# penn-graphics-research/HOT

Measured on AMD Instinct MI355X. Metric: ms per nonlinear (L-BFGS) iteration; P2G+G2P Mparticles/s; achieved HBM GB/s vs roofline, lower is better.
Workload: dtype f64; 1 GPU; C2: one 63^3-cell cube x 8 ppc (63^3 cells per GPU), fixed-corotated E=50000 nu=0.3, dx=0.01, dt=1/24, -lsolver 3 -mg_level 3 -smoother 5 -coarseSolver 2 --project --linesearch --bcproject --usecn -cneps 1e-7; particles_per_gpu=2000376, particles_total=2000376, nodes_total=267563, levels=3, parallelism=1 GPU

## Files before the change

hot_amd/csrc/mg_gs.hip:

```cpp
#include "hot_impl.h"

namespace hot {

#ifdef HOT_AB_KERNELS
#include "ab_src/mg_gs_ab1.hip"
#endif

template <class T, int SB>
struct GsLds {
    static constexpr int TRI = SB * (SB - 1) / 2 + 1;
    static constexpr size_t bytes = (size_t)9 * TRI * sizeof(T) + SB * 3 * sizeof(T) + 5 * SB * sizeof(int32_t);
};
template <class T>
struct GsWinv {
    static constexpr int img_elems = (9 * GsLds<T, 64>::TRI + 15) / 16 * 16;
};
template <int SB>
__device__ __forceinline__ int gs_tri_fwd(int row, int colm) { return (SB - 1) * colm - (colm * (colm - 1)) / 2 + (row - colm - 1); }
__device__ __forceinline__ int gs_tri_bwd(int row, int colm) { return (colm * (colm - 1)) / 2 + row; }
template <bool FWD>
__device__ __forceinline__ int gs_winv_idx(int row, int colm) { return FWD ? (row * (row - 1)) / 2 + colm : ((63 - row) * (62 - row)) / 2 + (63 - colm); }

template <class T>
__device__ __forceinline__ void gs_store_tri(T* tri, int TRI, int idx, const T* __restrict__ di, const T (&b)[9])
{
#pragma unroll
    for (int c = 0; c < 3; ++c)
#pragma unroll
        for (int r = 0; r < 3; ++r) tri[(r + 3 * c) * TRI + idx] = -(di[r] * b[3 * c] + di[r + 3] * b[3 * c + 1] + di[r + 6] * b[3 * c + 2]);
}
template <class T>
__device__ __forceinline__ void gs_store_rhs(T* sv, int ii, const T* __restrict__ di, T r0, T r1, T r2)
{
#pragma unroll
    for (int r = 0; r < 3; ++r) sv[ii * 3 + r] = di[r] * r0 + di[r + 3] * r1 + di[r + 6] * r2;
}

template <class T>
__global__ __launch_bounds__(1024) void k_gs_winv(const int32_t* __restrict__ col, const T* __restrict__ val, const uint32_t* __restrict__ ckey, const int32_t* __restrict__ gs_order,
    const int32_t* __restrict__ block_start, const int32_t* __restrict__ rowcnt, const T* __restrict__ diagBlockInv, const T* __restrict__ diagVal, T* __restrict__ gs_w)
{
    extern __shared__ __attribute__((aligned(16))) char gs_smem[];
    constexpr int TRI = GsLds<T, 64>::TRI;
    T* tri = (T*)gs_smem;
    T* sDi = tri + 9 * TRI;
    T* sDv = sDi + 64 * 9;
    int32_t* nodes = (int32_t*)(sDv + 64 * 9);
    const int tid = threadIdx.x, lane = tid & 63, w = tid >> 6, b = blockIdx.x;
    const int start = block_start[b], cnt = min(64, block_start[b + 1] - start);
    for (int e = tid; e < 9 * TRI; e += 1024) tri[e] = (T)0;
    if (tid < 64) nodes[tid] = tid < cnt ? gs_order[start + tid] : -1;
    __syncthreads();
    for (int e = tid; e < 9 * cnt; e += 1024) {
        const int64_t i = nodes[e / 9];
        sDi[e] = diagBlockInv[9 * i + e % 9], sDv[e] = diagVal[9 * i + e % 9];
    }
    for (int e = tid; e < 64 * cnt; e += 1024) {
        const int ii = e >> 6, ks = e & 63;
        const int64_t i = nodes[ii];
        const int po = rowcnt[4 * i], pi = rowcnt[4 * i + 1];
        if (ks >= pi) continue;
        const int k = po + ks, j = col[i * 125 + k];
        const int l = (int)(ckey[j] & 127u) - 1;
        T bb[9];
#pragma unroll
        for (int q = 0; q < 9; ++q) bb[q] = val[(i * 125 + k) * 9 + q];
        gs_store_tri<T>(tri, TRI, gs_tri_fwd<64>(ii, l), diagBlockInv + 9 * i, bb);
    }
    __syncthreads();
    T* outf = gs_w + ((size_t)b * 2) * GsWinv<T>::img_elems;
    T* outb = outf + GsWinv<T>::img_elems;
    if (tid < 9) outf[tid * TRI + TRI - 1] = (T)0, outb[tid * TRI + TRI - 1] = (T)0;
    for (int k4 = 0; k4 < 4; ++k4) {
        const int c0 = w + 16 * k4;
        if (c0 >= cnt) break;
        T a[3][3];
#pragma unroll
        for (int s_ = 0; s_ < 3; ++s_)
#pragma unroll
            for (int q = 0; q < 3; ++q) a[s_][q] = (lane == c0 && s_ == q) ? (T)1 : (T)0;
        for (int c = c0; c < cnt - 1; ++c) {
            const bool act = lane > c && lane < cnt;
            const int idx = act ? gs_tri_fwd<64>(lane, c) : TRI - 1;
            T Lc[9];
#pragma unroll
            for (int e = 0; e < 9; ++e) Lc[e] = tri[e * TRI + idx];
#pragma unroll
            for (int s_ = 0; s_ < 3; ++s_) {
                const T b0 = lane_bcast(a[s_][0], c), b1 = lane_bcast(a[s_][1], c), b2 = lane_bcast(a[s_][2], c);
                a[s_][0] = fma(Lc[0], b0, a[s_][0]), a[s_][1] = fma(Lc[1], b0, a[s_][1]), a[s_][2] = fma(Lc[2], b0, a[s_][2]);
                a[s_][0] = fma(Lc[3], b1, a[s_][0]), a[s_][1] = fma(Lc[4], b1, a[s_][1]), a[s_][2] = fma(Lc[5], b1, a[s_][2]);
                a[s_][0] = fma(Lc[6], b2, a[s_][0]), a[s_][1] = fma(Lc[7], b2, a[s_][1]), a[s_][2] = fma(Lc[8], b2, a[s_][2]);
            }
        }
        if (lane > c0 && lane < cnt) {
            const int idx = gs_winv_idx<true>(lane, c0);
#pragma unroll
            for (int s_ = 0; s_ < 3; ++s_)
#pragma unroll
                for (int q = 0; q < 3; ++q) outf[(q + 3 * s_) * TRI + idx] = a[s_][q];
        }
    }
    __threadfence();
    __syncthreads();
    for (int e = tid; e < 64 * 64; e += 1024) {
        const int r = e >> 6, c = e & 63;
        if (c <= r || c >= cnt) continue;
        const int fi = gs_winv_idx<true>(c, r), bi = gs_winv_idx<false>(r, c);
        T M[9], T1[9];
#pragma unroll
        for (int q = 0; q < 9; ++q) M[q] = __builtin_nontemporal_load(outf + q * TRI + fi);
        const T* Dc = sDv + 9 * c;
        const T* Ir = sDi + 9 * r;
#pragma unroll
        for (int j = 0; j < 3; ++j)
#pragma unroll
            for (int i = 0; i < 3; ++i) T1[i + 3 * j] = M[3 * i] * Dc[3 * j] + M[1 + 3 * i] * Dc[1 + 3 * j] + M[2 + 3 * i] * Dc[2 + 3 * j];
#pragma unroll
        for (int j = 0; j < 3; ++j)
#pragma unroll
            for (int i = 0; i < 3; ++i) outb[(i + 3 * j) * TRI + bi] = Ir[i] * T1[3 * j] + Ir[i + 3] * T1[1 + 3 * j] + Ir[i + 6] * T1[2 + 3 * j];
    }
}
template <class T>
void Ctx<T>::build_gs_winv(Level<T>& L)
{
    constexpr size_t per = 2 * (size_t)GsWinv<T>::img_elems;
    L.gs_w.reserve(per * (size_t)L.nblocks + 256);
    const size_t lds = ((size_t)9 * GsLds<T, 64>::TRI + 2 * 64 * 9) * sizeof(T) + 64 * sizeof(int32_t);
    if (!attr_winv_set) {
        HOT_HIP(hipFuncSetAttribute((const void*)k_gs_winv<T>, hipFuncAttributeMaxDynamicSharedMemorySize, (int)lds));
        attr_winv_set = true;
    }
    HOT_LAUNCH(this, lname("gs_winv", L.id).c_str(), k_gs_winv<T>, L.nblocks, 1024, lds, L.col.p, L.val.p, L.ckey.p, L.gs_order.p, L.gs_block_start.p, L.rowcnt.p, L.diagBlockInv.p, L.diagVal.p, L.gs_w.p);
    L.gs_w_ready = true;
}

template <class T, bool FWD, int SB, bool WT = false>
__device__ __forceinline__ void gs_phase_b(const T* tri, const T* sv, const int32_t* nodes, int cnt, int lane, const T* __restrict__ diagVal, const T* __restrict__ diagBlockInv, T* x, T* hD,
    const T* ldsD = nullptr);

#ifdef HOT_AB_KERNELS
__device__ int gs_dbg_flags = 0;
#define GS_DBG(bit) (gs_dbg_flags & (bit))
#else
#define GS_DBG(bit) 0
#endif
template <class T, bool FWD, int SB>
__global__ __launch_bounds__(1024) __attribute__((amdgpu_waves_per_eu(6))) void k_gs_block(const int32_t* __restrict__ col, const T* __restrict__ val, const uint32_t* __restrict__ ckey, const int32_t* __restrict__ gs_order,
    const int32_t* __restrict__ block_start, const T* __restrict__ diagVal, const T* __restrict__ diagBlockInv, const T* __restrict__ rhs, T* x, T* hD, int block0, int sub,
    const int32_t* __restrict__ rowcnt, const int32_t* __restrict__ gs_pad)
{
    extern __shared__ __attribute__((aligned(16))) char gs_smem[];
    constexpr int TRI = GsLds<T, SB>::TRI;
    T* tri = (T*)gs_smem;
    T* sv = tri + 9 * TRI;
    int32_t* nodes = (int32_t*)(sv + 3 * SB);
    int32_t* rcl = nodes + SB;
    const int tid = threadIdx.x, lane = tid & 63, w = tid >> 6;
    const int b = block0 + blockIdx.x;
    const int nmerge = max(sub >> 16, 1), sub_first = sub & 255;
    const int nthreads = blockDim.x, nwaves = blockDim.x >> 6;
    for (int m = 0; m < nmerge; ++m) {
    sub = FWD ? sub_first + m : sub_first + nmerge - 1 - m;
    const int lo = sub * SB;
    const int start = block_start[b] + lo, cnt = min(SB, block_start[b + 1] - start);
    if (cnt <= 0) continue;
    if (m > 0) __syncthreads();
    for (int e = tid; e < 9 * TRI; e += nthreads) tri[e] = (T)0;
    if (tid < SB) {
        const int4 rec0 = *(const int4*)(gs_pad + 8 * ((int64_t)b * 64 + lo + tid));
        const int rec1 = gs_pad[8 * ((int64_t)b * 64 + lo + tid) + 4];
        nodes[tid] = rec0.x;
        rcl[4 * tid] = rec0.y, rcl[4 * tid + 1] = rec0.z, rcl[4 * tid + 2] = rec0.w, rcl[4 * tid + 3] = rec1;
    }
    __syncthreads();
    constexpr int RQ = 2;
    for (int t0 = 0; w + nwaves * t0 < cnt && !GS_DBG(8); t0 += RQ) {
        T bv[RQ][9];
        int jj[RQ], rowi[RQ], kb[RQ], ke[RQ], ib[RQ], ie[RQ];
#pragma unroll
        for (int q = 0; q < RQ; ++q) {
            const int ii = w + nwaves * (t0 + q);
            rowi[q] = -1, jj[q] = -1, kb[q] = ke[q] = ib[q] = ie[q] = 0;
#pragma unroll
            for (int e = 0; e < 9; ++e) bv[q][e] = (T)0;
            if (ii < cnt) {
                const int i = __builtin_amdgcn_readfirstlane(nodes[ii]);
                rowi[q] = i;
                const int po = rcl[4 * ii], pi = rcl[4 * ii + 1], fi = rcl[4 * ii + 2], fo = rcl[4 * ii + 3];
                const int kbeg = FWD ? 0 : po + pi + 1, kend = FWD ? po + pi : po + pi + 1 + fi + fo;
                kb[q] = kbeg, ke[q] = kend, ib[q] = FWD ? po : kbeg, ie[q] = FWD ? po + pi : kbeg + fi;
                const int k = kbeg + lane, kc = max(min(k, kend - 1), 0);
                const int jl = col[(int64_t)i * 125 + kc];
                const T* bb = val + ((int64_t)i * 125 + kc) * 9;
                if (!GS_DBG(4)) {
#pragma unroll
                    for (int e = 0; e < 9; ++e) bv[q][e] = bb[e];
                }
                jj[q] = k < kend ? jl : -1;
            }
        }
#pragma unroll
        for (int q = 0; q < RQ; ++q) {
            const int i = rowi[q], ii = w + nwaves * (t0 + q);
            if (i < 0) continue;
            T di[9];
#pragma unroll
            for (int e = 0; e < 9; ++e) di[e] = diagBlockInv[9 * (int64_t)i + e];
            const T rh0 = rhs[3 * (int64_t)i], rh1 = rhs[3 * (int64_t)i + 1], rh2 = rhs[3 * (int64_t)i + 2];
            T s0 = 0, s1 = 0, s2 = 0;
            auto entry = [&](int k, int j, const T (&b9)[9]) {
                int lj = -1;
                if (k >= ib[q] && k < ie[q]) {
                    const int l = (int)(ckey[j] & 127u) - 1 - lo;
                    if (l >= 0 && l < SB) lj = l;
                }
                if (lj >= 0)
                    gs_store_tri<T>(tri, TRI, FWD ? gs_tri_fwd<SB>(ii, lj) : gs_tri_bwd(ii, lj), di, b9);
                else {
                    const T x0 = GS_DBG(2) ? (T)1 : x[3 * (int64_t)j], x1 = GS_DBG(2) ? (T)1 : x[3 * (int64_t)j + 1], x2 = GS_DBG(2) ? (T)1 : x[3 * (int64_t)j + 2];
                    s0 += b9[0] * x0 + b9[3] * x1 + b9[6] * x2;
                    s1 += b9[1] * x0 + b9[4] * x1 + b9[7] * x2;
                    s2 += b9[2] * x0 + b9[5] * x1 + b9[8] * x2;
                }
            };
            if (jj[q] >= 0) entry(kb[q] + lane, jj[q], bv[q]);
            for (int k = kb[q] + 64 + lane; k < ke[q]; k += 64) {
                T bt[9];
#pragma unroll
                for (int e = 0; e < 9; ++e) bt[e] = val[((int64_t)i * 125 + k) * 9 + e];
                entry(k, col[(int64_t)i * 125 + k], bt);
            }
            s0 = wave_sum(s0), s1 = wave_sum(s1), s2 = wave_sum(s2);
            if (lane == 0) gs_store_rhs<T>(sv, ii, di, rh0 - s0, rh1 - s1, rh2 - s2);
        }
    }
    __syncthreads();
    if (w == 0 && !GS_DBG(1)) gs_phase_b<T, FWD, SB>(tri, sv, nodes, cnt, lane, diagVal, diagBlockInv, x, hD);
    }
}

template <class T, bool FWD, int SB, bool WT>
__device__ __forceinline__ void gs_phase_b(const T* tri, const T* sv, const int32_t* nodes, int cnt, int lane, const T* __restrict__ diagVal, const T* __restrict__ diagBlockInv, T* x, T* hD,
    const T* ldsD)
{
    constexpr int TRI = GsLds<T, SB>::TRI;
    const int me = lane;
    const int i = me < cnt ? nodes[me] : -1;
    T a0 = me < cnt ? sv[me * 3] : (T)0, a1 = me < cnt ? sv[me * 3 + 1] : (T)0, a2 = me < cnt ? sv[me * 3 + 2] : (T)0;
    auto load_col = [&](int cidx, T (&L)[9]) {
        bool act = FWD ? (me > cidx && me < cnt) : (me < cidx);
        int idx = act ? (FWD ? gs_tri_fwd<SB>(me, cidx) : gs_tri_bwd(me, cidx)) : TRI - 1;
#pragma unroll
        for (int e = 0; e < 9; ++e) L[e] = tri[e * TRI + idx];
    };
    auto step = [&](int cidx, const T (&L)[9]) {
        T b0 = lane_bcast(a0, cidx), b1 = lane_bcast(a1, cidx), b2 = lane_bcast(a2, cidx);
        a0 = fma(L[0], b0, a0), a1 = fma(L[1], b0, a1), a2 = fma(L[2], b0, a2);
        a0 = fma(L[3], b1, a0), a1 = fma(L[4], b1, a1), a2 = fma(L[5], b1, a2);
        a0 = fma(L[6], b2, a0), a1 = fma(L[7], b2, a1), a2 = fma(L[8], b2, a2);
    };
    auto colof = [&](int s) { return FWD ? s : cnt - 1 - s; };
    T LA[9], LB[9];
    if (cnt > 0) load_col(colof(0), LA);
    int s = 0;
    for (; s + 1 < cnt; s += 2) {
        load_col(colof(s + 1), LB);
        step(colof(s), LA);
        load_col(colof(min(s + 2, cnt - 1)), LA);
        step(colof(s + 1), LB);
    }
    if (s < cnt) step(colof(s), LA);
    const T h0 = a0, h1 = a1, h2 = a2;
    T dd[9];
    if (FWD) {
#pragma unroll
        for (int e = 0; e < 9; ++e) dd[e] = i >= 0 ? (ldsD ? ldsD[9 * me + e] : diagVal[9 * (int64_t)i + e]) : (T)0;
    }
    if (i >= 0) {
        if (WT) {
            __hip_atomic_store(x + 3 * (int64_t)i, h0, __ATOMIC_RELAXED, __HIP_MEMORY_SCOPE_AGENT);
            __hip_atomic_store(x + 3 * (int64_t)i + 1, h1, __ATOMIC_RELAXED, __HIP_MEMORY_SCOPE_AGENT);
            __hip_atomic_store(x + 3 * (int64_t)i + 2, h2, __ATOMIC_RELAXED, __HIP_MEMORY_SCOPE_AGENT);
        }
        else
            x[3 * (int64_t)i] = h0, x[3 * (int64_t)i + 1] = h1, x[3 * (int64_t)i + 2] = h2;
        if (FWD) {
            hD[3 * (int64_t)i] = dd[0] * h0 + dd[3] * h1 + dd[6] * h2;
            hD[3 * (int64_t)i + 1] = dd[1] * h0 + dd[4] * h1 + dd[7] * h2;
            hD[3 * (int64_t)i + 2] = dd[2] * h0 + dd[5] * h1 + dd[8] * h2;
        }
        else if (hD) {
            hD[3 * (int64_t)i] += h0, hD[3 * (int64_t)i + 1] += h1, hD[3 * (int64_t)i + 2] += h2;
        }
    }
}

template <class T>
__device__ __forceinline__ T row16_sum(T v)
{
    v += dpp_move<0xb1, 0xf>(v);
    v += dpp_move<0x4e, 0xf>(v);
    v += dpp_move<0x114, 0xf>(v);
    v += dpp_move<0x118, 0xf>(v);
    return v;
}
template <class T>
struct GsOffItem {
    int j;
    bool valid;
    T bv[9];
};
template <class T, class Store>
__device__ __forceinline__ void gs_off_steps(const int2* __restrict__ slot, const int32_t* __restrict__ gcol, const T* __restrict__ val, const T* x, int s_begin, int s_end, int w, int W, int nstep, Store store)
{
    const int lane = threadIdx.x & 63, g = lane >> 4, l16 = lane & 15;
    if (w >= nstep) return;
    auto descriptor = [&](int n) __attribute__((always_inline)) {
        return slot[min(s_begin + 4 * min(n, nstep - 1) + g, s_end - 1)];
    };
    auto values = [&](int n, const int2 d, GsOffItem<T>& R) __attribute__((always_inline)) {
        R.valid = n < nstep && s_begin + 4 * n + g < s_end && l16 < d.y;
        const int64_t e = (int64_t)d.x + (R.valid ? l16 : 0);
        R.j = nt_load(gcol + e);
        const T* bb = val + e * 9;
#pragma unroll
        for (int t = 0; t < 9; ++t) R.bv[t] = nt_load(bb + t);
    };
    auto finish = [&](int n, const GsOffItem<T>& R, int nn, const int2 dn, GsOffItem<T>& N, int nd, int2& dd) __attribute__((always_inline)) {
        const int64_t jj = R.j;
        const T x0 = x[3 * jj], x1 = x[3 * jj + 1], x2 = x[3 * jj + 2];
        asm volatile("" ::: "memory");
        values(nn, dn, N);
        dd = descriptor(nd);
        asm volatile("" ::: "memory");
        const T(&b)[9] = R.bv;
        T s[3] = { b[0] * x0 + b[3] * x1 + b[6] * x2, b[1] * x0 + b[4] * x1 + b[7] * x2, b[2] * x0 + b[5] * x1 + b[8] * x2 };
#pragma unroll
        for (int d = 0; d < 3; ++d) s[d] = row16_sum(R.valid ? s[d] : (T)0);
        const int sl = s_begin + 4 * n + g;
        if (l16 == 15 && n < nstep && sl < s_end) store(sl, s[0], s[1], s[2]);
    };
    GsOffItem<T> A, B;
    int2 d1 = descriptor(w + W), d2;
    values(w, descriptor(w), A);
    d2 = descriptor(w + 2 * W);
    asm volatile("" ::: "memory");
    for (int n = w; n < nstep; n += 2 * W) {
        int2 d3, d4;
        finish(n, A, n + W, d1, B, n + 3 * W, d3);
        finish(n + W, B, n + 2 * W, d2, A, n + 4 * W, d4);
        d1 = d3, d2 = d4;
    }
}
template <class T>
__device__ __forceinline__ void gs_off_stream(const int2* __restrict__ slot, const int32_t* __restrict__ gcol, const T* __restrict__ val, const T* x, T* part, int s_begin, int s_end, int bid, int nwg)
{
    const int nstep_all = (s_end - s_begin + 3) >> 2;
    const bool by_xcd = (nwg & 7) == 0;
    const int chunk = by_xcd ? (nstep_all + 7) >> 3 : nstep_all, xcd = by_xcd ? (bid & 7) : 0;
    const int W = by_xcd ? (nwg >> 3) * 4 : nwg * 4;
    const int nstep = min(nstep_all, (xcd + 1) * chunk);
    const int w = __builtin_amdgcn_readfirstlane(xcd * chunk + (int)((by_xcd ? bid >> 3 : bid) * 4 + (threadIdx.x >> 6)));
    gs_off_steps<T>(slot, gcol, val, x, s_begin, s_end, w, W, nstep, [&](int sl, T s0, T s1, T s2) __attribute__((always_inline)) {
        T* o = part + 3 * (int64_t)sl;
        o[0] = s0, o[1] = s1, o[2] = s2;
    });
}
template <class T>
__global__ __launch_bounds__(256) void k_gs_offblock(const int2* __restrict__ slot, const int32_t* __restrict__ gcol, const T* __restrict__ val, const int32_t* __restrict__ gs_pad,
    const T* __restrict__ x, T* __restrict__ part, int s_begin, int s_end )
{
    gs_off_stream<T>(slot, gcol, val, x, part, s_begin, s_end, (int)blockIdx.x, (int)gridDim.x);
}

template <class T, bool FWD, int D>
__global__ __launch_bounds__(64) void k_gs_subst(const T* __restrict__ img, const uint16_t* __restrict__ imgi, const int32_t* __restrict__ gs_pad, const T* __restrict__ part, T* x,
    T* hD, int block0, const T* __restrict__ rhs, T* hsub )
{
    using I = GsImg<T>;
    const int lane = threadIdx.x;
    const int b = block0 + blockIdx.x;
    const T* hdr = img + (size_t)b * I::per_block;
    const T* ent = hdr + I::hdr_elems + (FWD ? 0 : I::per_dir);
    const int64_t pos = (int64_t)b * 64 + lane;
    const int32_t* rec = gs_pad + 8 * pos;
    const int node = rec[0], nslot = ((FWD ? rec[1] : rec[4]) + 15) >> 4, slot0 = rec[FWD ? 5 : 6];
    uint32_t iw[32];
    {
        const uint4* ip = (const uint4*)(imgi + ((size_t)b * 2 + (FWD ? 0 : 1)) * I::idx_per_dir + lane * 64);
#pragma unroll
        for (int q = 0; q < 8; ++q) {
            const uint4 v = ip[q];
            iw[4 * q] = v.x, iw[4 * q + 1] = v.y, iw[4 * q + 2] = v.z, iw[4 * q + 3] = v.w;
        }
    }
    T ring[D][9];
#define HOT_GS_ISSUE(s, L)                                                                   \
    do {                                                                                      \
        const uint32_t idx_ = (iw[(s) >> 1] >> (16 * ((s)&1))) & 0xffffu;                     \
        const T* p_ = ent + (size_t)idx_ * 9;                                                 \
        _Pragma("unroll") for (int e_ = 0; e_ < 9; ++e_) L[e_] = p_[e_];                      \
        asm volatile("" ::: "memory");  \
    } while (0)
#pragma unroll
    for (int k = 0; k < D; ++k) HOT_GS_ISSUE(k, ring[k]);
    T a0, a1, a2;
    {
        const T* src = rhs + 3 * (int64_t)max(node, 0);
        T q0 = src[0], q1 = src[1], q2 = src[2];
        T ps[8][3];
#pragma unroll
        for (int q = 0; q < 8; ++q) {
            const T* pp = part + 3 * (int64_t)(slot0 + (q < nslot ? q : 0));
            ps[q][0] = pp[0], ps[q][1] = pp[1], ps[q][2] = pp[2];
        }
        T s0 = 0, s1 = 0, s2 = 0;
#pragma unroll
        for (int q = 0; q < 8; ++q) s0 += q < nslot ? ps[q][0] : (T)0, s1 += q < nslot ? ps[q][1] : (T)0, s2 += q < nslot ? ps[q][2] : (T)0;
        q0 -= s0, q1 -= s1, q2 -= s2;
        const T* di = hdr + 576 + 9 * lane;
        a0 = di[0] * q0 + di[3] * q1 + di[6] * q2, a1 = di[1] * q0 + di[4] * q1 + di[7] * q2, a2 = di[2] * q0 + di[5] * q1 + di[8] * q2;
    }
    T dd[9];
    if (FWD) {
#pragma unroll
        for (int e = 0; e < 9; ++e) dd[e] = hdr[9 * lane + e];
    }
#pragma unroll
    for (int s = 0; s < 64; ++s) {
        const int c = FWD ? s : 63 - s;
        const T b0 = lane_bcast(a0, c), b1 = lane_bcast(a1, c), b2 = lane_bcast(a2, c);
        T(&L)[9] = ring[s % D];
        a0 = fma(L[0], b0, a0), a1 = fma(L[1], b0, a1), a2 = fma(L[2], b0, a2);
        a0 = fma(L[3], b1, a0), a1 = fma(L[4], b1, a1), a2 = fma(L[5], b1, a2);
        a0 = fma(L[6], b2, a0), a1 = fma(L[7], b2, a1), a2 = fma(L[8], b2, a2);
        if (s + D < 64) HOT_GS_ISSUE(s + D, L);
    }
#undef HOT_GS_ISSUE
    if (node < 0) return;
    x[3 * (int64_t)node] = a0, x[3 * (int64_t)node + 1] = a1, x[3 * (int64_t)node + 2] = a2;
    if (FWD) {
        hD[3 * (int64_t)node] = dd[0] * a0 + dd[3] * a1 + dd[6] * a2;
        hD[3 * (int64_t)node + 1] = dd[1] * a0 + dd[4] * a1 + dd[7] * a2;
        hD[3 * (int64_t)node + 2] = dd[2] * a0 + dd[5] * a1 + dd[8] * a2;
    }
    else {
        if (hD) hD[3 * (int64_t)node] += a0, hD[3 * (int64_t)node + 1] += a1, hD[3 * (int64_t)node + 2] += a2;
        if (hsub) hsub[3 * (int64_t)node] -= a0, hsub[3 * (int64_t)node + 1] -= a1, hsub[3 * (int64_t)node + 2] -= a2;
    }
}

#ifdef HOT_GSC_CLOCKS
__device__ unsigned long long gsc_clk[16][12];
__device__ unsigned long long gsc_blk[4096][8];
__device__ unsigned long long gsc_str[4096][2];
__global__ void k_gsc_pass(int p, int nb, int ns)
{
    __shared__ unsigned long long red[8][256], lo[2][256], hi[2][256];
    const int t = threadIdx.x;
    unsigned long long a[8] = {}, l0 = ~0ull, h0 = 0, l1 = ~0ull, h1 = 0;
    for (int i = t; i < nb && i < 4096; i += 256) {
        for (int k = 0; k < 6; ++k) a[k] += gsc_blk[i][k];
        l0 = min(l0, gsc_blk[i][6]), h0 = max(h0, gsc_blk[i][7]);
    }
    for (int i = t; i < ns && i < 4096; i += 256) l1 = min(l1, gsc_str[i][0]), h1 = max(h1, gsc_str[i][1]);
    for (int k = 0; k < 6; ++k) red[k][t] = a[k];
    lo[0][t] = l0, hi[0][t] = h0, lo[1][t] = l1, hi[1][t] = h1;
    __syncthreads();
    if (t == 0) {
        for (int i = 1; i < 256; ++i) {
            for (int k = 0; k < 6; ++k) red[k][0] += red[k][i];
            lo[0][0] = min(lo[0][0], lo[0][i]), hi[0][0] = max(hi[0][0], hi[0][i]), lo[1][0] = min(lo[1][0], lo[1][i]), hi[1][0] = max(hi[1][0], hi[1][i]);
        }
        unsigned long long* c = gsc_clk[p];
        c[0] += (unsigned long long)nb;
        for (int k = 0; k < 5; ++k) c[1 + k] += red[k][0];
        c[7] += red[5][0];
        if (nb > 0 && hi[0][0] > lo[0][0]) c[6] += hi[0][0] - lo[0][0];
        if (ns > 0 && hi[1][0] > lo[1][0]) c[8] += hi[1][0] - lo[1][0];
        c[9] += 1;
    }
}
#define HOT_GS_CLK(i)                                  \
    do {                                               \
        asm volatile("" ::: "memory");                 \
        const unsigned long long t_ = wall_clock64();  \
        clk_[i] = t_ - tl_, tl_ = t_;                  \
        asm volatile("" ::: "memory");                 \
    } while (0)
#else
#define HOT_GS_CLK(i)
#endif
template <class T, bool FWD, int D, bool TURN = false>
__global__ __launch_bounds__(256) void k_gs_colour(const T* __restrict__ img, const uint16_t* __restrict__ imgi, const int32_t* __restrict__ gs_pad, const int4* __restrict__ srec, T* x, T* hD, int block0,
    int nb, int nb_pad , const T* __restrict__ rhs, T* hsub, const int2* __restrict__ slot,
    const int32_t* __restrict__ gcol, const T* __restrict__ val, T* part, int s_begin, int s_end ,
    T* xb , T* ub )
{
    static_assert(!TURN || FWD, "the turn is the end of the forward sweep");
#ifdef HOT_GSC_CLOCKS
    const unsigned long long t00_ = wall_clock64();
    unsigned long long tl_ = t00_, clk_[6] = {};
#endif
    if ((int)blockIdx.x >= nb_pad) {
        gs_off_stream<T>(slot, gcol, val, x, part, s_begin, s_end, (int)blockIdx.x - nb_pad, (int)gridDim.x - nb_pad);
#ifdef HOT_GSC_CLOCKS
        const int sid_ = (int)blockIdx.x - nb_pad;
        if (threadIdx.x == 0 && sid_ < 4096) gsc_str[sid_][0] = t00_, gsc_str[sid_][1] = wall_clock64();
#endif
        return;
    }
    if ((int)blockIdx.x >= nb) return;
    using I = GsImg<T>;
    __shared__ T lprev[3 * 512];
    __shared__ T ldv[9 * 64];
    __shared__ uint32_t lidx[(TURN ? 2 : 1) * 64 * 33];
    const int b = block0 + blockIdx.x;
    const int p0 = FWD ? srec[(int64_t)b * 64].y : srec[(int64_t)b * 64].w, p1 = FWD ? srec[(int64_t)b * 64 + 64].y : srec[(int64_t)b * 64 + 64].w;
    const int wave = threadIdx.x >> 6, lane = threadIdx.x & 63;
    const T* hdr = img + (size_t)b * I::per_block;
    if (wave != 0) {
        gs_off_steps<T>(slot, gcol, val, x, p0, p1, wave - 1, 3, (p1 - p0 + 3) >> 2, [&](int sl, T s0, T s1, T s2) __attribute__((always_inline)) {
            T* o = lprev + 3 * (sl - p0);
            o[0] = s0, o[1] = s1, o[2] = s2;
        });
#ifdef HOT_GSC_CLOCKS
        if (threadIdx.x == 64 && blockIdx.x < 4096) gsc_blk[blockIdx.x][5] = wall_clock64() - t00_;
#endif
        __syncthreads();
        return;
    }
    const T* ent = hdr + I::hdr_elems + (FWD ? 0 : I::per_dir);
    const int64_t pos = (int64_t)b * 64 + lane;
    const int4 r0 = *(const int4*)(gs_pad + 8 * pos), r1 = *(const int4*)(gs_pad + 8 * pos + 4), sr = srec[pos];
    {
        const uint4* ip = (const uint4*)(imgi + ((size_t)b * 2 + (FWD ? 0 : 1)) * I::idx_per_dir + lane * 64);
        uint4 v[8];
#pragma unroll
        for (int q = 0; q < 8; ++q) v[q] = ip[q];
#pragma unroll
        for (int q = 0; q < 8; ++q) lidx[33 * lane + 4 * q] = v[q].x, lidx[33 * lane + 4 * q + 1] = v[q].y, lidx[33 * lane + 4 * q + 2] = v[q].z, lidx[33 * lane + 4 * q + 3] = v[q].w;
        if (TURN) {
            const uint4* ipb = (const uint4*)(imgi + ((size_t)b * 2 + 1) * I::idx_per_dir + lane * 64);
#pragma unroll
            for (int q = 0; q < 8; ++q) v[q] = ipb[q];
#pragma unroll
            for (int q = 0; q < 8; ++q)
                lidx[64 * 33 + 33 * lane + 4 * q] = v[q].x, lidx[64 * 33 + 33 * lane + 4 * q + 1] = v[q].y, lidx[64 * 33 + 33 * lane + 4 * q + 2] = v[q].z, lidx[64 * 33 + 33 * lane + 4 * q + 3] = v[q].w;
        }
    }
    const int node = r0.x, nall = FWD ? r0.y : r1.x, nprev_e = FWD ? (r1.w & 0xffff) : ((r1.w >> 16) & 0xffff);
    const int nold = (nall - nprev_e + 15) >> 4, nprev = (nprev_e + 15) >> 4, so = FWD ? sr.x : sr.z, sp = (FWD ? sr.y : sr.w) - p0;
    T q0, q1, q2;
    {
        const T* src = rhs + 3 * (int64_t)max(node, 0);
        q0 = src[0], q1 = src[1], q2 = src[2];
        T ps[8][3];
#pragma unroll
        for (int q = 0; q < 8; ++q) {
            const T* pp = part + 3 * (int64_t)(so + (q < nold ? q : 0));
            ps[q][0] = pp[0], ps[q][1] = pp[1], ps[q][2] = pp[2];
        }
        const T* di = hdr + 576 + 9 * lane;
#pragma unroll
        for (int e = 0; e < 9; ++e) ldv[64 * e + lane] = di[e];
        T s0 = 0, s1 = 0, s2 = 0;
#pragma unroll
        for (int q = 0; q < 8; ++q) s0 += q < nold ? ps[q][0] : (T)0, s1 += q < nold ? ps[q][1] : (T)0, s2 += q < nold ? ps[q][2] : (T)0;
        q0 -= s0, q1 -= s1, q2 -= s2;
        asm volatile("" : "+v"(q0), "+v"(q1), "+v"(q2)::"memory");
    }
    HOT_GS_CLK(0);
    const uint16_t* lrow = (const uint16_t*)(lidx + 33 * lane);
    T ring[D][9];
#define HOT_GS_ISSUE(E, LR, s, L)                                                            \
    do {                                                                                      \
        const uint32_t idx_ = (LR)[s];                                                        \
        const T* p_ = (E) + (size_t)idx_ * 9;                                                 \
        _Pragma("unroll") for (int e_ = 0; e_ < 9; ++e_) L[e_] = nt_load(p_ + e_);            \
        asm volatile("" ::: "memory");  \
    } while (0)
#pragma unroll
    for (int k = 0; k < D; ++k) HOT_GS_ISSUE(ent, lrow, k, ring[k]);
    HOT_GS_CLK(1);
    __syncthreads();
    HOT_GS_CLK(2);
    T a0, a1, a2;
    {
        T s0 = 0, s1 = 0, s2 = 0;
#pragma unroll
        for (int q = 0; q < 8; ++q) {
            const T* pp = lprev + 3 * (q < nprev ? sp + q : 0);
            const T v0 = pp[0], v1 = pp[1], v2 = pp[2];
            s0 += q < nprev ? v0 : (T)0, s1 += q < nprev ? v1 : (T)0, s2 += q < nprev ? v2 : (T)0;
            if (q & 1) asm volatile("" : "+v"(s0), "+v"(s1), "+v"(s2));
        }
        q0 -= s0, q1 -= s1, q2 -= s2;
        a0 = ldv[lane] * q0 + ldv[64 * 3 + lane] * q1 + ldv[64 * 6 + lane] * q2;
        asm volatile("" : "+v"(a0));
        a1 = ldv[64 + lane] * q0 + ldv[64 * 4 + lane] * q1 + ldv[64 * 7 + lane] * q2;
        asm volatile("" : "+v"(a1));
        a2 = ldv[64 * 2 + lane] * q0 + ldv[64 * 5 + lane] * q1 + ldv[64 * 8 + lane] * q2;
    }
    T dd[9];
    const T* entb = hdr + I::hdr_elems + I::per_dir;
    const uint16_t* lrowb = (const uint16_t*)(lidx + 64 * 33 + 33 * lane);
#pragma unroll
    for (int s = 0; s < 64; ++s) {
        const int c = FWD ? s : 63 - s;
        const T b0 = lane_bcast(a0, c), b1 = lane_bcast(a1, c), b2 = lane_bcast(a2, c);
        T(&L)[9] = ring[s % D];
        a0 = fma(L[0], b0, a0), a1 = fma(L[1], b0, a1), a2 = fma(L[2], b0, a2);
        a0 = fma(L[3], b1, a0), a1 = fma(L[4], b1, a1), a2 = fma(L[5], b1, a2);
        a0 = fma(L[6], b2, a0), a1 = fma(L[7], b2, a1), a2 = fma(L[8], b2, a2);
        if (s + D < 64) HOT_GS_ISSUE(ent, lrow, s + D, L);
        else if (TURN) HOT_GS_ISSUE(entb, lrowb, s + D - 64, L);
        if (FWD && s + D == 64) {
#pragma unroll
            for (int e = 0; e < 9; ++e) dd[e] = hdr[9 * lane + e];
            asm volatile("" ::: "memory");
        }
    }
#ifdef HOT_GSC_CLOCKS
    asm volatile("" : "+v"(a0), "+v"(a1), "+v"(a2)::"memory");
    HOT_GS_CLK(3);
    auto clk_out = [&]() __attribute__((always_inline)) {
        HOT_GS_CLK(4);
        if (lane == 0) {
            if (blockIdx.x < 4096) {
                for (int i = 0; i < 5; ++i) gsc_blk[blockIdx.x][i] = clk_[i];
                gsc_blk[blockIdx.x][6] = t00_, gsc_blk[blockIdx.x][7] = tl_;
            }
        }
    };
#endif
    if (!TURN && node < 0) return;
    T h0 = 0, h1 = 0, h2 = 0;
    if (FWD) {
        h0 = dd[0] * a0 + dd[3] * a1 + dd[6] * a2, h1 = dd[1] * a0 + dd[4] * a1 + dd[7] * a2, h2 = dd[2] * a0 + dd[5] * a1 + dd[8] * a2;
        if (node >= 0) {
            if (!TURN) x[3 * (int64_t)node] = a0, x[3 * (int64_t)node + 1] = a1, x[3 * (int64_t)node + 2] = a2;
            hD[3 * (int64_t)node] = h0, hD[3 * (int64_t)node + 1] = h1, hD[3 * (int64_t)node + 2] = h2;
        }
    }
    else {
        x[3 * (int64_t)node] = a0, x[3 * (int64_t)node + 1] = a1, x[3 * (int64_t)node + 2] = a2;
        if (hD) hD[3 * (int64_t)node] += a0, hD[3 * (int64_t)node + 1] += a1, hD[3 * (int64_t)node + 2] += a2;
        if (hsub) hsub[3 * (int64_t)node] -= a0, hsub[3 * (int64_t)node + 1] -= a1, hsub[3 * (int64_t)node + 2] -= a2;
    }
    if constexpr (TURN) {
        const T f0 = a0, f1 = a1, f2 = a2;
        a0 = ldv[lane] * h0 + ldv[64 * 3 + lane] * h1 + ldv[64 * 6 + lane] * h2;
        asm volatile("" : "+v"(a0));
        a1 = ldv[64 + lane] * h0 + ldv[64 * 4 + lane] * h1 + ldv[64 * 7 + lane] * h2;
        asm volatile("" : "+v"(a1));
        a2 = ldv[64 * 2 + lane] * h0 + ldv[64 * 5 + lane] * h1 + ldv[64 * 8 + lane] * h2;
#pragma unroll
        for (int s = 0; s < 64; ++s) {
            const int c = 63 - s;
            const T b0 = lane_bcast(a0, c), b1 = lane_bcast(a1, c), b2 = lane_bcast(a2, c);
            T(&L)[9] = ring[(64 + s) % D];
            a0 = fma(L[0], b0, a0), a1 = fma(L[1], b0, a1), a2 = fma(L[2], b0, a2);
            a0 = fma(L[3], b1, a0), a1 = fma(L[4], b1, a1), a2 = fma(L[5], b1, a2);
            a0 = fma(L[6], b2, a0), a1 = fma(L[7], b2, a1), a2 = fma(L[8], b2, a2);
            if (s + D < 64) HOT_GS_ISSUE(entb, lrowb, s + D, L);
        }
        if (node < 0) return;
        xb[3 * (int64_t)node] = a0, xb[3 * (int64_t)node + 1] = a1, xb[3 * (int64_t)node + 2] = a2;
        if (ub) ub[3 * (int64_t)node] += a0, ub[3 * (int64_t)node + 1] += a1, ub[3 * (int64_t)node + 2] += a2;
        if (hsub)
            x[3 * (int64_t)node] = f0 - a0, x[3 * (int64_t)node + 1] = f1 - a1, x[3 * (int64_t)node + 2] = f2 - a2;
        else
            x[3 * (int64_t)node] = f0, x[3 * (int64_t)node + 1] = f1, x[3 * (int64_t)node + 2] = f2;
    }
#ifdef HOT_GSC_CLOCKS
    if (!TURN) clk_out();
#endif
#undef HOT_GS_ISSUE
}

template <class T>
__global__ void k_gs_fill_unset(size_t n, T* x)
{
    const size_t i = (size_t)blockIdx.x * blockDim.x + threadIdx.x;
    if (i >= n) return;
    if constexpr (sizeof(T) == 8)
        ((unsigned long long*)x)[i] = GsUnset<double>::bits;
    else
        ((unsigned*)x)[i] = GsUnset<float>::bits;
}
struct GsPasses {
    int npass;
    int wg_begin[34];
    int block0[33];
    int sub[33];
    int color[33];
};

#ifdef HOT_GS_CLOCKS
__device__ unsigned long long gs_clk[34 * 8];
#define GS_CLK(i) \
    do { \
        const unsigned long long t_ = clock64(); \
        gclk_[i] += t_ - gt0_, gt0_ = t_; \
    } while (0)
#else
#define GS_CLK(i)
#endif
template <class T, bool FWD, int SB, bool WINV = false>
__global__ __launch_bounds__(SB * 16) void k_gs_sweep(const int32_t* __restrict__ col, const T* __restrict__ val, const uint32_t* __restrict__ ckey, const int32_t* __restrict__ gs_order,
    const int32_t* __restrict__ block_start, const T* __restrict__ diagVal, const T* __restrict__ diagBlockInv, const T* __restrict__ rhs, T* x, T* hD, GsPasses P,
    const int32_t* __restrict__ rowcnt, int* err ,
    T* unset_next ,
    const T* __restrict__ gs_w )
{
    extern __shared__ __attribute__((aligned(16))) char gs_smem[];
    constexpr int TRI = GsLds<T, SB>::TRI;
    static_assert(!WINV || SB == 64, "the inverse images are whole-block images");
#ifdef HOT_GS_CLOCKS
    unsigned long long gclk_[5] = { 0, 0, 0, 0, 0 }, gt0_ = clock64();
#endif
    constexpr int RQ = 4, NW = SB / RQ;
    auto ld3 = [&](int64_t j, T& x0, T& x1, T& x2) {
        x0 = __hip_atomic_load(x + 3 * j, __ATOMIC_RELAXED, __HIP_MEMORY_SCOPE_AGENT), x1 = __hip_atomic_load(x + 3 * j + 1, __ATOMIC_RELAXED, __HIP_MEMORY_SCOPE_AGENT),
        x2 = __hip_atomic_load(x + 3 * j + 2, __ATOMIC_RELAXED, __HIP_MEMORY_SCOPE_AGENT);
        int spins = 0;
        while (GsUnset<T>::is(x0) || GsUnset<T>::is(x1) || GsUnset<T>::is(x2)) {
            __builtin_amdgcn_s_sleep(2);
            if (++spins > (1 << 21) || ((spins & 1023) == 0 && *(volatile int*)err)) {
                *(volatile int*)err = 1;
                break;
            }
            x0 = __hip_atomic_load(x + 3 * j, __ATOMIC_RELAXED, __HIP_MEMORY_SCOPE_AGENT), x1 = __hip_atomic_load(x + 3 * j + 1, __ATOMIC_RELAXED, __HIP_MEMORY_SCOPE_AGENT),
            x2 = __hip_atomic_load(x + 3 * j + 2, __ATOMIC_RELAXED, __HIP_MEMORY_SCOPE_AGENT);
        }
    };
    T* tri = (T*)gs_smem;
    T* sv = tri + (WINV ? GsWinv<T>::img_elems : 9 * TRI);
    int32_t* nodes = (int32_t*)(sv + 3 * SB);
    const int tid = threadIdx.x, lane = tid & 63, w = tid >> 6;
    int p = 0;
    while (p + 1 < P.npass && (int)blockIdx.x >= P.wg_begin[p + 1]) ++p;
    const int b = P.block0[p] + ((int)blockIdx.x - P.wg_begin[p]);
    const int lo = P.sub[p] * SB;
    const int start = block_start[b] + lo, cnt = max(0, min(SB, block_start[b + 1] - start));
    int32_t* rng = nodes + SB;
    T* sDinv = (T*)(nodes + 5 * SB);
    T* sD = sDinv + 9 * SB;
    T* srhs = sD + 9 * SB;
    if (!WINV)
        for (int e = tid; e < 9 * TRI; e += 64 * NW) tri[e] = (T)0;
    if (tid < SB) nodes[tid] = tid < cnt ? gs_order[start + tid] : -1;
    __syncthreads();
    GS_CLK(0);
    if (WINV) {
        constexpr int IMG_BYTES = GsWinv<T>::img_elems * (int)sizeof(T);
        const char* wg = (const char*)(gs_w + ((size_t)b * 2 + (FWD ? 0 : 1)) * GsWinv<T>::img_elems);
        for (int c = w; c * 1024 < IMG_BYTES; c += NW) {
            const int off = c * 1024 + lane * 16;
            if (off < IMG_BYTES)
                __builtin_amdgcn_global_load_lds((const __attribute__((address_space(1))) void*)(wg + off), (__attribute__((address_space(3))) void*)((char*)tri + c * 1024), 16, 0, 0);
        }
    }
    for (int e = tid; e < 9 * cnt; e += 64 * NW) {
        const int64_t i = nodes[e / 9];
        sDinv[e] = diagBlockInv[9 * i + e % 9];
        if (FWD) sD[e] = diagVal[9 * i + e % 9];
    }
    for (int e = tid; e < 3 * cnt; e += 64 * NW) srhs[e] = rhs[3 * (int64_t)nodes[e / 3] + e % 3];
    if (unset_next)
        for (int e = tid; e < 3 * cnt; e += 64 * NW) gs_store_unset(unset_next + 3 * (int64_t)nodes[e / 3] + e % 3);
    T bv[RQ][9];
    int jj[RQ], node[RQ], kb2[RQ], ke[RQ];
    const bool first_sub = p == 0 || P.color[p - 1] != P.color[p];
    const bool head = FWD ? first_sub : !first_sub;
    bool late[RQ];
    const uint32_t prevkey = p > 0 ? ((uint32_t)P.color[p - 1] << 8) | (uint32_t)P.sub[p - 1] : 0xffffffffu;
    if constexpr (WINV) {
        int4 rc[RQ];
#pragma unroll
        for (int q = 0; q < RQ; ++q) {
            const int ii = w + NW * q;
            jj[q] = -1, kb2[q] = 0, ke[q] = 0, late[q] = false;
            node[q] = ii < cnt ? __builtin_amdgcn_readfirstlane(nodes[ii]) : -1;
#pragma unroll
            for (int e = 0; e < 9; ++e) bv[q][e] = (T)0;
        }
#pragma unroll
        for (int q = 0; q < RQ; ++q) rc[q] = node[q] >= 0 ? *(const int4*)(rowcnt + 4 * (int64_t)node[q]) : make_int4(0, 0, 0, 0);
#pragma unroll
        for (int q = 0; q < RQ; ++q) {
            if (node[q] < 0) continue;
            const int64_t i = node[q];
            const int kbeg = FWD ? 0 : rc[q].x + rc[q].y + 1 + rc[q].z, kend = FWD ? rc[q].x : kbeg + rc[q].w;
            kb2[q] = head ? kbeg + 64 : kbeg, ke[q] = head ? kend : kend - 64;
            const int k = head ? kbeg + lane : kend - 64 + lane;
            if (k >= kbeg && k < kend) {
                jj[q] = col[i * 125 + k];
                const T* bb = val + (i * 125 + k) * 9;
#pragma unroll
                for (int e = 0; e < 9; ++e) bv[q][e] = bb[e];
            }
        }
#pragma unroll
        for (int q = 0; q < RQ; ++q)
            if (jj[q] >= 0) {
                const uint32_t keyj = ckey[jj[q]];
                late[q] = (((keyj >> 28) << 8) | (((keyj & 127u) - 1u) / (uint32_t)SB)) == prevkey;
            }
    }
    else
#pragma unroll
    for (int q = 0; q < RQ; ++q) {
        const int ii = w + NW * q;
        jj[q] = -1, node[q] = -1, kb2[q] = 0, ke[q] = 0, late[q] = false;
#pragma unroll
        for (int e = 0; e < 9; ++e) bv[q][e] = (T)0;
        if (ii < cnt) {
            const int i = nodes[ii];
            node[q] = i;
            const int po = rowcnt[4 * i], pi = rowcnt[4 * i + 1], fi = rowcnt[4 * i + 2], fo = rowcnt[4 * i + 3];
            const int kbeg = FWD ? 0 : po + pi + 1, kend = FWD ? po + pi : po + pi + 1 + fi + fo;
            const int ibeg = FWD ? po : kbeg, iend = FWD ? po + pi : kbeg + fi;
            kb2[q] = head ? kbeg + 64 : kbeg, ke[q] = head ? kend : kend - 64;
            rng[ii] = kb2[q], rng[SB + ii] = ke[q];
            const int k = head ? kbeg + lane : kend - 64 + lane;
            if (k >= kbeg && k < kend) {
                const int j = col[(int64_t)i * 125 + k];
                const T* bb = val + ((int64_t)i * 125 + k) * 9;
#pragma unroll
                for (int e = 0; e < 9; ++e) bv[q][e] = bb[e];
                jj[q] = j;
                const uint32_t keyj = ckey[j];
                late[q] = (((keyj >> 28) << 8) | (((keyj & 127u) - 1u) / (uint32_t)SB)) == prevkey;
                if (k >= ibeg && k < iend) {
                    const int l = (int)(keyj & 127u) - 1 - lo;
                    if (l >= 0 && l < SB) {
                        if (!WINV) {
                            const int idx = FWD ? gs_tri_fwd<SB>(ii, l) : gs_tri_bwd(ii, l);
                            gs_store_tri<T>(tri, TRI, idx, diagBlockInv + 9 * (int64_t)i, bv[q]);
                        }
                        jj[q] = -1;
                    }
                }
            }
        }
    }
    __syncthreads();
    GS_CLK(1);
    auto is_late = [&](uint32_t keyj) { return (((keyj >> 28) << 8) | (((keyj & 127u) - 1u) / (uint32_t)SB)) == prevkey; };
    bool tail_late[RQ];
#pragma unroll
    for (int q = 0; q < RQ; ++q) {
        const int ii = w + NW * q;
        tail_late[q] = false;
        if (ii >= cnt) continue;
        const int i = WINV ? node[q] : nodes[ii], kt0 = WINV ? kb2[q] : rng[ii], kt1 = WINV ? ke[q] : rng[SB + ii];
        T e0 = 0, e1 = 0, e2 = 0;
        if (jj[q] >= 0 && !late[q]) {
            const int64_t j = jj[q];
            T x0, x1, x2;
            ld3(j, x0, x1, x2);
            e0 = bv[q][0] * x0 + bv[q][3] * x1 + bv[q][6] * x2;
            e1 = bv[q][1] * x0 + bv[q][4] * x1 + bv[q][7] * x2;
            e2 = bv[q][2] * x0 + bv[q][5] * x1 + bv[q][8] * x2;
        }
        bool tl = false;
        for (int k = kt0 + lane; k < kt1; k += 64) {
            const int j = col[(int64_t)i * 125 + k];
            const T* bb = val + ((int64_t)i * 125 + k) * 9;
            const uint32_t keyj = ckey[j], keyi = ckey[i];
            const int l = (int)(keyj & 127u) - 1 - lo;
            if ((keyj >> 7) == (keyi >> 7) && l >= 0 && l < SB) {
                if (!WINV) {
                    const int idx = FWD ? gs_tri_fwd<SB>(ii, l) : gs_tri_bwd(ii, l);
                    T bt[9];
#pragma unroll
                    for (int e = 0; e < 9; ++e) bt[e] = bb[e];
                    gs_store_tri<T>(tri, TRI, idx, diagBlockInv + 9 * (int64_t)i, bt);
                }
            }
            else if (is_late(keyj))
                tl = true;
            else {
                T x0, x1, x2;
                ld3(j, x0, x1, x2);
                e0 += bb[0] * x0 + bb[3] * x1 + bb[6] * x2;
                e1 += bb[1] * x0 + bb[4] * x1 + bb[7] * x2;
                e2 += bb[2] * x0 + bb[5] * x1 + bb[8] * x2;
            }
        }
        tail_late[q] = __ballot(tl) != 0ull;
        e0 = wave_sum(e0), e1 = wave_sum(e1), e2 = wave_sum(e2);
        if (lane == 0) srhs[3 * ii] -= e0, srhs[3 * ii + 1] -= e1, srhs[3 * ii + 2] -= e2;
    }
    GS_CLK(2);
    const T* val_again = val;
    asm volatile("" : "+s"(val_again));
#pragma unroll
    for (int q = 0; q < RQ; ++q) {
        const int ii = w + NW * q;
        if (ii >= cnt) continue;
        const int i = WINV ? node[q] : nodes[ii], kt0 = WINV ? kb2[q] : rng[ii], kt1 = WINV ? ke[q] : rng[SB + ii];
        T s0 = 0, s1 = 0, s2 = 0;
        if (jj[q] >= 0 && late[q]) {
            const int64_t j = jj[q];
            const T* bb = val_again + ((int64_t)i * 125 + (head ? kt0 - 64 : kt1) + lane) * 9;
            T bl[9];
#pragma unroll
            for (int e = 0; e < 9; ++e) bl[e] = bb[e];
            T x0, x1, x2;
            ld3(j, x0, x1, x2);
            s0 = bl[0] * x0 + bl[3] * x1 + bl[6] * x2;
            s1 = bl[1] * x0 + bl[4] * x1 + bl[7] * x2;
            s2 = bl[2] * x0 + bl[5] * x1 + bl[8] * x2;
        }
        if (tail_late[q]) {
            for (int k = kt0 + lane; k < kt1; k += 64) {
                const int j = col[(int64_t)i * 125 + k];
                const T* bb = val + ((int64_t)i * 125 + k) * 9;
                const uint32_t keyj = ckey[j], keyi = ckey[i];
                const int l = (int)(keyj & 127u) - 1 - lo;
                if (!((keyj >> 7) == (keyi >> 7) && l >= 0 && l < SB) && is_late(keyj)) {
                    T x0, x1, x2;
                    ld3(j, x0, x1, x2);
                    s0 += bb[0] * x0 + bb[3] * x1 + bb[6] * x2;
                    s1 += bb[1] * x0 + bb[4] * x1 + bb[7] * x2;
                    s2 += bb[2] * x0 + bb[5] * x1 + bb[8] * x2;
                }
            }
        }
        s0 = wave_sum(s0), s1 = wave_sum(s1), s2 = wave_sum(s2);
        if (lane == 0) gs_store_rhs<T>(sv, ii, sDinv + 9 * ii, srhs[3 * ii] - s0, srhs[3 * ii + 1] - s1, srhs[3 * ii + 2] - s2);
    }
    __syncthreads();
    GS_CLK(3);
#ifdef HOT_GS_CLOCKS
#define GS_CLK_OUT() \
    do { \
        GS_CLK(4); \
        if (tid == 0) \
            for (int i = 0; i < 5; ++i) atomicAdd(&gs_clk[p * 8 + i], gclk_[i]); \
        if (tid == 0) atomicAdd(&gs_clk[p * 8 + 7], 1ull); \
    } while (0)
#else
#define GS_CLK_OUT()
#endif
    if (WINV) {
        const bool cin = lane < cnt;
        const T ac0 = cin ? sv[3 * lane] : (T)0, ac1 = cin ? sv[3 * lane + 1] : (T)0, ac2 = cin ? sv[3 * lane + 2] : (T)0;
        T h0 = 0, h1 = 0, h2 = 0;
#pragma unroll
        for (int k = 0; k < 4; ++k) {
            const int rr = 4 * w + k;
            if (rr >= cnt) break;
            const bool act = FWD ? lane < rr : (lane > rr && cin);
            const int idx = act ? gs_winv_idx<FWD>(rr, lane) : TRI - 1;
            T Lw[9];
#pragma unroll
            for (int e = 0; e < 9; ++e) Lw[e] = tri[e * TRI + idx];
            T t0 = Lw[0] * ac0 + Lw[3] * ac1 + Lw[6] * ac2, t1 = Lw[1] * ac0 + Lw[4] * ac1 + Lw[7] * ac2, t2 = Lw[2] * ac0 + Lw[5] * ac1 + Lw[8] * ac2;
            t0 = wave_sum(t0), t1 = wave_sum(t1), t2 = wave_sum(t2);
            if (lane == k) h0 = sv[3 * rr] + t0, h1 = sv[3 * rr + 1] + t1, h2 = sv[3 * rr + 2] + t2;
        }
        const int me = 4 * w + lane;
        if (lane < 4 && me < cnt) {
            const int64_t i = nodes[me];
            __hip_atomic_store(x + 3 * i, h0, __ATOMIC_RELAXED, __HIP_MEMORY_SCOPE_AGENT);
            __hip_atomic_store(x + 3 * i + 1, h1, __ATOMIC_RELAXED, __HIP_MEMORY_SCOPE_AGENT);
            __hip_atomic_store(x + 3 * i + 2, h2, __ATOMIC_RELAXED, __HIP_MEMORY_SCOPE_AGENT);
            if (FWD) {
                const T* dd = sD + 9 * me;
                hD[3 * i] = dd[0] * h0 + dd[3] * h1 + dd[6] * h2, hD[3 * i + 1] = dd[1] * h0 + dd[4] * h1 + dd[7] * h2, hD[3 * i + 2] = dd[2] * h0 + dd[5] * h1 + dd[8] * h2;
            }
            else if (hD)
                hD[3 * i] += h0, hD[3 * i + 1] += h1, hD[3 * i + 2] += h2;
        }
        GS_CLK_OUT();
        return;
    }
    if (w != 0) return;
    if (cnt > 0) gs_phase_b<T, FWD, SB, true>(tri, sv, nodes, cnt, lane, diagVal, diagBlockInv, x, hD, sD);
    GS_CLK_OUT();
}

template <class T>
__global__ void k_gs_hdiff(size_t n3, T* __restrict__ h, const T* __restrict__ du)
{
    const size_t i = (size_t)blockIdx.x * blockDim.x + threadIdx.x;
    if (i < n3) h[i] -= du[i];
}
template <class T, bool DIFF = false>
__global__ __launch_bounds__(256) void k_gs_residual(const int32_t* __restrict__ col, const T* __restrict__ val, const int32_t* __restrict__ rowcnt, const T* __restrict__ h,
    const T* __restrict__ du, T* __restrict__ r, int n, const uint8_t* __restrict__ own, const uint8_t* __restrict__ owner ,
    int me, const T* __restrict__ l1e )
{
    const int lane = threadIdx.x & 63;
    const int row = xcd_block() * 4 + (threadIdx.x >> 6);
    if (row >= n || (own && !own[row])) return;
    const int nl = rowcnt[4 * row] + rowcnt[4 * row + 1];
    const int32_t* c = col + (int64_t)row * 125;
    const T* v = val + (int64_t)row * 1125;
    T s0 = 0, s1 = 0, s2 = 0;
    auto add = [&](int k, int j) {
        const T* b = v + k * 9;
        T x0 = h[3 * (int64_t)j], x1 = h[3 * (int64_t)j + 1], x2 = h[3 * (int64_t)j + 2];
        if (!DIFF) x0 -= du[3 * (int64_t)j], x1 -= du[3 * (int64_t)j + 1], x2 -= du[3 * (int64_t)j + 2];
        s0 += b[0] * x0 + b[3] * x1 + b[6] * x2;
        s1 += b[1] * x0 + b[4] * x1 + b[7] * x2;
        s2 += b[2] * x0 + b[5] * x1 + b[8] * x2;
    };
    {
        const int q = lane / 3, cc = lane - 3 * q;
        for (int base = 0; base < nl; base += 63)
#pragma unroll
        for (int k0 = 0; k0 < 63; k0 += 21) {
            const int k = base + k0 + q;
            const bool ok = lane < 63 && k < nl;
            const int kk = ok ? k : 0;
            const int64_t j = nt_load(c + kk);
            const T* b = v + kk * 9 + 3 * cc;
            const T b0 = nt_load(b), b1 = nt_load(b + 1), b2 = nt_load(b + 2);
            T x = h[3 * j + cc];
            if (!DIFF) x -= du[3 * j + cc];
            x = ok ? x : (T)0;
            s0 += b0 * x, s1 += b1 * x, s2 += b2 * x;
        }
    }
    if (owner) {
        const int ub = nl + 1 + rowcnt[4 * row + 2], ue = ub + rowcnt[4 * row + 3];
        for (int k = ub + lane; k < ue; k += 64) {
            const int j = c[k];
            if (owner[j] != me) add(k, j);
        }
    }
    s0 = wave_sum(s0), s1 = wave_sum(s1), s2 = wave_sum(s2);
    if (lane == 0) {
        if (l1e) s0 += l1e[3 * (int64_t)row] * du[3 * (int64_t)row], s1 += l1e[3 * (int64_t)row + 1] * du[3 * (int64_t)row + 1], s2 += l1e[3 * (int64_t)row + 2] * du[3 * (int64_t)row + 2];
        r[3 * (int64_t)row] = s0, r[3 * (int64_t)row + 1] = s1, r[3 * (int64_t)row + 2] = s2;
    }
}

template <class T>
static int max_colour_blocks(const Level<T>& L)
{
    int max_nb = 0;
    for (int c = 0; c < 8; ++c) max_nb = std::max(max_nb, L.color_block_begin[c + 1] - L.color_block_begin[c]);
    return max_nb;
}
template <class T>
static bool chain_allowed(const Ctx<T>& ctx, const Level<T>& L, int max_nb)
{
    return !ctx.gs_no_chain && ctx.cfg.gs_chain != 1 && !L.part && (ctx.cfg.gs_chain == 2 || max_nb <= 256);
}
template <class T>
GsPlan Ctx<T>::gs_plan(const Level<T>& L) const
{
    const int max_nb = max_colour_blocks(L);
    const bool simple_gs = ab_flag("HOT_SIMPLE_GS");
    const bool chained = chain_allowed(*this, L, max_nb) && !simple_gs && L.split;
    GsPlan p{};
    p.sb = cfg.gs_sub_block ? cfg.gs_sub_block : ((max_nb > 256 || (chained && max_nb > 32 && !L.gs_w_ready)) ? 32 : 64);
    p.nmerge = (ab_flag("HOT_GS_SPLIT_LAUNCHES") || simple_gs) ? 1 : 64 / p.sb;
    const bool images = p.sb == 32 && L.gs_img_ready && p.nmerge > 1 && !simple_gs && !ab_flag("HOT_GS_V1");
    if (chained)
        p.path = GsPlan::CHAINED;
    else if (images && L.gs_fused_ready && !L.part)
        p.path = GsPlan::COLOUR;
    else if (images)
        p.path = GsPlan::PAIR;
    else
        p.path = simple_gs ? GsPlan::SIMPLE : GsPlan::PER_COLOUR;
    if (chained) {
        p.winv = p.sb == 64 && L.gs_w_ready && !ab_flag("HOT_GS_NO_WINV");
        p.marks = L.tmp.p != nullptr;
    }
    return p;
}
template <class T>
GsBuild Ctx<T>::gs_build(const Level<T>& L) const
{
    const int max_nb = max_colour_blocks(L);
    GsBuild b{};
    b.winv = sizeof(T) == 8 && smoother_kind(L.id) == 5 && chain_allowed(*this, L, max_nb) && (cfg.gs_sub_block == 0 || cfg.gs_sub_block == 64) && L.nblocks <= 2048;
    b.images = max_nb > 256 || cfg.gs_sub_block == 32;
    b.colour_lists = !L.part && !ab_flag("HOT_GS_PAIR");
    return b;
}

template <class T>
static bool raise_gs_lds_limits(Ctx<T>& ctx)
{
    if (ctx.attr_gs_set) return false;
    HOT_HIP(hipFuncSetAttribute((const void*)k_gs_block<T, true, 64>, hipFuncAttributeMaxDynamicSharedMemorySize, (int)GsLds<T, 64>::bytes));
    HOT_HIP(hipFuncSetAttribute((const void*)k_gs_block<T, false, 64>, hipFuncAttributeMaxDynamicSharedMemorySize, (int)GsLds<T, 64>::bytes));
    HOT_HIP(hipFuncSetAttribute((const void*)k_gs_sweep<T, true, 64>, hipFuncAttributeMaxDynamicSharedMemorySize, (int)(GsLds<T, 64>::bytes + 21 * 64 * sizeof(T) + 128)));
    HOT_HIP(hipFuncSetAttribute((const void*)k_gs_sweep<T, false, 64>, hipFuncAttributeMaxDynamicSharedMemorySize, (int)(GsLds<T, 64>::bytes + 21 * 64 * sizeof(T) + 128)));
    HOT_HIP(hipFuncSetAttribute((const void*)k_gs_sweep<T, true, 64, true>, hipFuncAttributeMaxDynamicSharedMemorySize, (int)(GsLds<T, 64>::bytes + 21 * 64 * sizeof(T) + 128)));
    HOT_HIP(hipFuncSetAttribute((const void*)k_gs_sweep<T, false, 64, true>, hipFuncAttributeMaxDynamicSharedMemorySize, (int)(GsLds<T, 64>::bytes + 21 * 64 * sizeof(T) + 128)));
    ctx.attr_gs_set = true;
    return true;
}
template <class T>
struct ExchangeAfterColour {
    Ctx<T>* ctx;
    Level<T>& L;
    T* x;
    int c;
    bool on;
    ~ExchangeAfterColour()
    {
        if (on) ctx->exchange(L, x, c);
    }
};

template <class T>
void Ctx<T>::ic_smooth_dev(Level<T>& L, T* u, T* r, T* dAu)
{
    HOT_CHECK(L.ic_ready && L.split, HOT_ERR_INVALID, "coarseSolver 7: the level has no incomplete-Cholesky factor (hot_build_mg)");
    raise_gs_lds_limits(*this);
    T* y = L.tmp.p;
    for (int c = 0; c < 8; ++c) {
        const int b0 = L.color_block_begin[c], nb = L.color_block_begin[c + 1] - b0;
        if (nb > 0)
            HOT_LAUNCH(this, lname("ic_forward", L.id).c_str(), (k_gs_block<T, true, 64>), nb, 1024, (GsLds<T, 64>::bytes), L.ic_col.p, L.ic_val.p, L.ckey.p, L.gs_order.p, L.gs_block_start.p,
                L.ic_d.p, L.ic_dinv.p, r, y, dAu, b0, 0 | (1 << 16), L.ic_rowcnt.p, L.ic_pad.p);
    }
    for (int c = 7; c >= 0; --c) {
        const int b0 = L.color_block_begin[c], nb = L.color_block_begin[c + 1] - b0;
        if (nb > 0)
            HOT_LAUNCH(this, lname("ic_backward", L.id).c_str(), (k_gs_block<T, false, 64>), nb, 1024, (GsLds<T, 64>::bytes), L.ic_col.p, L.ic_val.p, L.ckey.p, L.gs_order.p, L.gs_block_start.p,
                L.ic_d.p, L.ic_dinvT.p, y, u, (T*)nullptr, b0, 0 | (1 << 16), L.ic_rowcnt.p, L.ic_pad.p);
    }
}

template <class T>
void Ctx<T>::gs_smooth_dev(int level, int iterations, T* u, T* r, T* du, T* dAu, bool final_residual, bool tmp_marked)
{
    Level<T>& L = *levels[level];
    const size_t n3 = 3 * (size_t)L.n;
    const bool hm = L.part && halo_mode();
    HOT_CHECK(L.nblocks > 0, HOT_ERR_INVALID, "GS smoother requested but the level was built without colouring");
    T* hdu = L.tmp.p;
    const bool rank_local = L.part && cfg.shard_gs != 0;
    const bool no_lres = ab_flag("HOT_GS_FULL_RESIDUAL");
    if (raise_gs_lds_limits(*this)) {
#ifdef HOT_AB_KERNELS
        if (const char* e = getenv("HOT_GS_DBG")) {
            const int f = atoi(e);
            HOT_HIP(hipMemcpyToSymbol(HIP_SYMBOL(gs_dbg_flags), &f, sizeof(int)));
        }
#endif
    }
    const GsPlan plan = gs_plan(L);
    const bool simple_gs = plan.path == GsPlan::SIMPLE;
    const int sb = plan.sb, nsub = 64 / sb, nmerge = plan.nmerge;
    HOT_CHECK(L.split || simple_gs, HOT_ERR_INVALID, "block GS kernels need the regrouped rows (k_gs_split_rows)");
    HOT_CHECK(sb == 16 || sb == 32 || sb == 64, HOT_ERR_INVALID, "hot_config.gs_sub_block must be 0 (auto), 16, 32 or 64");
    HOT_CHECK(cfg.gs_chain >= 0 && cfg.gs_chain <= 2, HOT_ERR_INVALID, "hot_config.gs_chain must be 0 (auto), 1 (one launch per colour) or 2 (one chained launch per half sweep)");

    auto pass = [&](bool fwd, int c, int h) {
        if (L.color_block_begin[c + 1] <= L.color_block_begin[c]) return;
        if (nmerge > 1 && h != 0) return;
        const char* nm = fwd ? "gs_forward" : "gs_backward";
        const T* rhs = fwd ? r : dAu;
        T* xx = fwd ? hdu : du;
        const int32_t* rc = L.rowcnt.p;
        ExchangeAfterColour<T> after{ this, L, xx, c, L.part && !rank_local && (nmerge > 1 || (fwd ? h == nsub - 1 : h == 0)) };
        const auto [b0, b1] = L.colour_run(c, comm.rank, comm.size);
        const int nb = b1 - b0;
        if (nb <= 0) return;
        T* hD = fwd ? dAu : ((simple_gs || L.part) ? (T*)nullptr : u);
#ifdef HOT_AB_KERNELS
        if (simple_gs) {
            if (h != 0) return;
            if (fwd)
                HOT_LAUNCH(this, lname(nm, L.id).c_str(), (k_gs_color<T, true>), nb, 64, 0, L.col.p, L.val.p, L.ckey.p, L.gs_order.p, L.gs_block_start.p, L.gs_d(), L.gs_dinv(), rhs, xx, hD, b0, nb);
            else
                HOT_LAUNCH(this, lname(nm, L.id).c_str(), (k_gs_color<T, false>), nb, 64, 0, L.col.p, L.val.p, L.ckey.p, L.gs_order.p, L.gs_block_start.p, L.gs_d(), L.gs_dinv(), rhs, xx, hD, b0, nb);
            return;
        }
#endif
        const int gs_threads = sb == 64 ? 1024 : 512;
#define HOT_GS_CASE(F, S)                                                                                                                                      \
    HOT_LAUNCH(this, lname(nm, L.id).c_str(), (k_gs_block<T, F, S>), nb, gs_threads, (GsLds<T, S>::bytes), L.col.p, L.val.p, L.ckey.p, L.gs_order.p, L.gs_block_start.p, \
        L.gs_d(), L.gs_dinv(), rhs, xx, hD, b0, h | (nmerge << 16), rc, L.gs_pad.p)
        if (fwd) {
            if (sb == 64) HOT_GS_CASE(true, 64);
            else if (sb == 32) HOT_GS_CASE(true, 32);
            else HOT_GS_CASE(true, 16);
        }
        else {
            if (sb == 64) HOT_GS_CASE(false, 64);
            else if (sb == 32) HOT_GS_CASE(false, 32);
            else HOT_GS_CASE(false, 16);
        }
#undef HOT_GS_CASE
    };
    auto per_colour_sweep = [&](bool fwd) {
        if (fwd)
            for (int c = 0; c < 8; ++c)
                for (int h = 0; h < nsub; ++h) pass(true, c, h);
        else
            for (int c = 7; c >= 0; --c)
                for (int h = nsub - 1; h >= 0; --h) pass(false, c, h);
    };

    auto pair_sweep = [&](bool fwd) {
        const T* rhs = fwd ? r : dAu;
        T* xx = fwd ? hdu : du;
        T* hD = fwd ? dAu : u;
        const char* nmT = fwd ? "gs_forward" : "gs_backward";
        const char* nmO = fwd ? "gs_forward_off" : "gs_backward_off";
        T* hsub = (!fwd && !L.part) ? hdu : (T*)nullptr;
        if (L.part) hD = fwd ? dAu : (T*)nullptr;
        for (int q = 0; q < 8; ++q) {
            const int c = fwd ? q : 7 - q;
            if (L.color_block_begin[c + 1] <= L.color_block_begin[c]) continue;
            ExchangeAfterColour<T> after{ this, L, xx, c, L.part && !rank_local };
            const auto [b0, b1] = L.colour_run(c, comm.rank, comm.size);
            const int nb = b1 - b0;
            if (nb <= 0) continue;
            const int s0 = L.gs_slot_rng[fwd ? 0 : 1][0][c], s1 = L.gs_slot_rng[fwd ? 0 : 1][1][c];
            const T* img_c = L.gs_img.p + L.gs_img_shift[c] * (long long)GsImg<T>::per_block;
            const uint16_t* imgi_c = L.gs_imgi.p + L.gs_img_shift[c] * 2 * (long long)GsImg<T>::idx_per_dir;
            const int grid = std::max(1, ab_int("HOT_GS_OFF_WAVES", 4096) / 4);
            if (s1 > s0) HOT_LAUNCH(this, lname(nmO, L.id).c_str(), k_gs_offblock<T>, grid, 256, 0, L.gs_slot.p, L.gs_col.p, L.val.p, L.gs_pad.p, xx, L.gs_p1.p, s0, s1);
#ifdef HOT_AB_KERNELS
            const int depth = ab_int("HOT_GS_SUBST_D", 8);
#define HOT_SUBST_D(DD)                                                                                                                                                       \
    if (depth == DD) {                                                                                                                                                        \
        if (fwd)                                                                                                                                                              \
            HOT_LAUNCH(this, lname(nmT, L.id).c_str(), (k_gs_subst<T, true, DD>), nb, 64, 0, img_c, imgi_c, L.gs_pad.p, L.gs_p1.p, xx, hD, b0, rhs, hsub);                 \
        else                                                                                                                                                                  \
            HOT_LAUNCH(this, lname(nmT, L.id).c_str(), (k_gs_subst<T, false, DD>), nb, 64, 0, img_c, imgi_c, L.gs_pad.p, L.gs_p1.p, xx, hD, b0, rhs, hsub);                \
        continue;                                                                                                                                                             \
    }
            HOT_SUBST_D(4)
            HOT_SUBST_D(6)
            HOT_SUBST_D(10)
            HOT_SUBST_D(12)
            HOT_SUBST_D(16)
#undef HOT_SUBST_D
#endif
            if (fwd)
                HOT_LAUNCH(this, lname(nmT, L.id).c_str(), (k_gs_subst<T, true, 8>), nb, 64, 0, img_c, imgi_c, L.gs_pad.p, L.gs_p1.p, xx, hD, b0, rhs, hsub);
            else
                HOT_LAUNCH(this, lname(nmT, L.id).c_str(), (k_gs_subst<T, false, 8>), nb, 64, 0, img_c, imgi_c, L.gs_pad.p, L.gs_p1.p, xx, hD, b0, rhs, hsub);
        }
    };

    const bool turn = !ab_flag("HOT_GS_NO_TURN");
    auto colour_sweep = [&](bool fwd) {
        const T* rhs = fwd ? r : dAu;
        T* xx = fwd ? hdu : du;
        T* hD = fwd ? dAu : u;
#ifndef HOT_AB_KERNELS
        const char* nm = fwd ? "gs_forward_fused" : "gs_backward_fused";
#endif
        T* hsub = !fwd ? hdu : (T*)nullptr;
        const int nstream = std::max(8, ab_int("HOT_GS_OFF_WAVES", 4096) / 4 / 8 * 8);
        int last = -1;
        for (int c = 7; c >= 0 && last < 0; --c)
            if (L.color_block_begin[c + 1] > L.color_block_begin[c]) last = c;
        for (int q = 0; q < 8; ++q) {
            const int c = fwd ? q : 7 - q, cn = fwd ? c + 1 : c - 1;
            const int b0 = L.color_block_begin[c], nb = L.color_block_begin[c + 1] - b0, nb_pad = (nb + 7) & ~7;
            const int s0 = (cn >= 0 && cn < 8) ? L.gs_slot_rng2[fwd ? 0 : 2][0][cn] : 0, s1 = (cn >= 0 && cn < 8) ? L.gs_slot_rng2[fwd ? 0 : 2][1][cn] : 0;
            const bool do_turn = turn && c == last && nb > 0;
            const int grid = (!fwd && do_turn ? 0 : nb_pad) + (s1 > s0 ? nstream : 0);
            if (grid == 0) continue;
            const int nbk = (!fwd && do_turn) ? 0 : nb, nbk_pad = (!fwd && do_turn) ? 0 : nb_pad;
#ifdef HOT_AB_KERNELS
            const std::string nmq = ab_flag("HOT_GS_PROF_COLOURS") ? std::string(fwd ? "gs_forward_fused_q" : "gs_backward_fused_q") + char('0' + q) : std::string(fwd ? "gs_forward_fused" : "gs_backward_fused");
            const char* nm = nmq.c_str();
#endif
#define HOT_COLOUR_D(DD)                                                                                                                                                       \
    do {                                                                                                                                                                       \
        if (fwd && do_turn)                                                                                                                                                    \
            HOT_LAUNCH(this, lname(nm, L.id).c_str(), (k_gs_colour<T, true, DD, true>), grid, 256, 0, L.gs_img.p, L.gs_imgi.p, L.gs_pad.p, L.gs_srec.p, xx, hD, b0, nbk, nbk_pad, rhs, \
                (!L.part ? hdu : (T*)nullptr), L.gs_slot.p, L.gs_col.p, L.val.p, L.gs_p1.p, s0, s1, du, u);                                                                       \
        else if (fwd)                                                                                                                                                          \
            HOT_LAUNCH(this, lname(nm, L.id).c_str(), (k_gs_colour<T, true, DD>), grid, 256, 0, L.gs_img.p, L.gs_imgi.p, L.gs_pad.p, L.gs_srec.p, xx, hD, b0, nbk, nbk_pad, rhs, hsub, \
                L.gs_slot.p, L.gs_col.p, L.val.p, L.gs_p1.p, s0, s1, (T*)nullptr, (T*)nullptr);                                                                                \
        else                                                                                                                                                                   \
            HOT_LAUNCH(this, lname(nm, L.id).c_str(), (k_gs_colour<T, false, DD>), grid, 256, 0, L.gs_img.p, L.gs_imgi.p, L.gs_pad.p, L.gs_srec.p, xx, hD, b0, nbk, nbk_pad, rhs, hsub, \
                L.gs_slot.p, L.gs_col.p, L.val.p, L.gs_p1.p, s0, s1, (T*)nullptr, (T*)nullptr);                                                                                \
    } while (0)
#ifdef HOT_AB_KERNELS
            const int depth = ab_int("HOT_GS_SUBST_D", 0);
            if (depth == 4) {
                HOT_COLOUR_D(4);
                continue;
            }
            if (depth == 6) {
                HOT_COLOUR_D(6);
                continue;
            }
            if (depth == 7) {
                HOT_COLOUR_D(7);
                continue;
            }
            if (depth == 8) {
                HOT_COLOUR_D(8);
                continue;
            }
#endif
            if constexpr (sizeof(T) == 8)
                HOT_COLOUR_D(7);
            else
                HOT_COLOUR_D(8);
#undef HOT_COLOUR_D
#ifdef HOT_GSC_CLOCKS
            if (L.id == 0) hipLaunchKernelGGL(k_gsc_pass, dim3(1), dim3(256), 0, stream, (fwd ? 0 : 8) + q, nbk, grid - nbk_pad);
#endif
        }
    };

    if (tmp_marked && !plan.marks) zero(n3, hdu), tmp_marked = false;
    GsPasses PF{}, PB{};
    if (plan.path == GsPlan::CHAINED) {
        auto add = [&](GsPasses& P, int c, int h) {
            int b0 = L.color_block_begin[c], nb = L.color_block_begin[c + 1] - b0;
            if (nb <= 0) return;
            P.block0[P.npass] = b0, P.sub[P.npass] = h, P.color[P.npass] = c, P.wg_begin[P.npass + 1] = P.wg_begin[P.npass] + nb;
            ++P.npass;
        };
        for (int c = 0; c < 8; ++c)
            for (int h = 0; h < nsub; ++h) add(PF, c, h);
        for (int c = 7; c >= 0; --c)
            for (int h = nsub - 1; h >= 0; --h) add(PB, c, h);
    }
    bool du_marked = false;
    auto chained_sweep = [&](bool fwd) {
        const GsPasses& P = fwd ? PF : PB;
        if (P.npass == 0) return;
        const char* nm = fwd ? "gs_forward" : "gs_backward";
        const T* rhs = fwd ? r : dAu;
        T* xx = fwd ? hdu : du;
        T* hD = fwd ? dAu : u;
        const int32_t* rc = L.rowcnt.p;
        const bool marked = fwd ? tmp_marked : du_marked;
        if (fwd) tmp_marked = false;
        if (!marked) HOT_LAUNCH(this, "gs_fill_unset", k_gs_fill_unset<T>, div_up(n3, 256), 256, 0, n3, xx);
        const int grid = P.wg_begin[P.npass];
#define HOT_GS_CASE(F, S, ...)                                                                                                                                         \
    HOT_LAUNCH(this, lname(nm, L.id).c_str(), (k_gs_sweep<T, F, S, ##__VA_ARGS__>), grid, 16 * S, (GsLds<T, S>::bytes + 21 * S * sizeof(T) + 128), L.col.p, L.val.p, L.ckey.p, L.gs_order.p, L.gs_block_start.p, \
        L.diagVal.p, L.diagBlockInv.p, rhs, xx, hD, P, rc, (int*)(hscal + 250), \
        fwd ? du : (T*)nullptr, L.gs_w.p)
        du_marked = fwd;
        if (plan.winv) {
            if (fwd)
                HOT_GS_CASE(true, 64, true);
            else
                HOT_GS_CASE(false, 64, true);
        }
        else if (fwd) {
            if (sb == 64) HOT_GS_CASE(true, 64);
            else if (sb == 32) HOT_GS_CASE(true, 32);
            else HOT_GS_CASE(true, 16);
        }
        else {
            if (sb == 64) HOT_GS_CASE(false, 64);
            else if (sb == 32) HOT_GS_CASE(false, 32);
            else HOT_GS_CASE(false, 16);
        }
#undef HOT_GS_CASE
    };
#ifdef HOT_GS_CLOCKS
    auto clk_report = [&](const char* what) {
        unsigned long long h[34 * 8];
        HOT_HIP(hipStreamSynchronize(stream));
        HOT_HIP(hipMemcpyFromSymbol(h, HIP_SYMBOL(gs_clk), sizeof(h)));
        if (h[7]) {
            fprintf(stderr, "k_gs_sweep %s level %d, clocks per workgroup [header, rows, early gathers, wait + late gathers, solve]:", what, L.id);
            for (int q = 0; q < 33 && h[q * 8 + 7]; ++q) fprintf(stderr, " | p%d(%llu wg) %.0f %.0f %.0f %.0f %.0f", q, h[q * 8 + 7], (double)h[q * 8] / h[q * 8 + 7], (double)h[q * 8 + 1] / h[q * 8 + 7], (double)h[q * 8 + 2] / h[q * 8 + 7], (double)h[q * 8 + 3] / h[q * 8 + 7], (double)h[q * 8 + 4] / h[q * 8 + 7]);
            fprintf(stderr, "\n");
        }
        memset(h, 0, sizeof(h));
        HOT_HIP(hipMemcpyToSymbol(HIP_SYMBOL(gs_clk), h, sizeof(h)));
    };
#endif
    auto half_sweep = [&](bool fwd) {
        switch (plan.path) {
        case GsPlan::CHAINED: chained_sweep(fwd); break;
        case GsPlan::COLOUR: colour_sweep(fwd); break;
        case GsPlan::PAIR: pair_sweep(fwd); break;
        case GsPlan::PER_COLOUR:
        case GsPlan::SIMPLE: per_colour_sweep(fwd); break;
        }
    };

    iterations = ((iterations + 1) >> 1);
    for (; iterations--;) {
        prof.count(lname("gs_symsweeps", L.id));
        if (rank_local) zero(n3, hdu), zero(n3, du);
        half_sweep(true);
#ifdef HOT_GS_CLOCKS
        if (plan.path == GsPlan::CHAINED) clk_report("forward");
#endif
        half_sweep(false);
#ifdef HOT_GSC_CLOCKS
        if (plan.path == GsPlan::COLOUR && L.id == 0) {
            static int sweeps = 0;
            if (++sweeps % 10 == 0) {
                unsigned long long h[16][12];
                HOT_HIP(hipStreamSynchronize(stream));
                HOT_HIP(hipMemcpyFromSymbol(h, HIP_SYMBOL(gsc_clk), sizeof(h)));
                fprintf(stderr, "k_gs_colour, per-role clocks (100 MHz), us: per block of the substitution wavefront | per launch\n"
                                "pass        blocks  trips1+2  requests  wait-prev  64-steps  stores | summing-done | block-wgs-span  stream-wgs-span\n");
                for (int p = 0; p < 16; ++p) {
                    if (!h[p][9] || !h[p][0]) continue;
                    const double nb = (double)h[p][0], nl = (double)h[p][9];
                    fprintf(stderr, "%s q%d  %7.0f  %8.2f  %8.2f  %9.2f  %8.2f  %6.2f | %12.2f | %14.2f  %15.2f\n", p < 8 ? "forward " : "backward", p & 7, nb / nl, h[p][1] / (100 * nb), h[p][2] / (100 * nb),
                        h[p][3] / (100 * nb), h[p][4] / (100 * nb), h[p][5] / (100 * nb), h[p][7] / (100 * nb), h[p][6] / (100 * nl), h[p][8] / (100 * nl));
                }
                memset(h, 0, sizeof(h));
                HOT_HIP(hipMemcpyToSymbol(HIP_SYMBOL(gsc_clk), h, sizeof(h)));
            }
        }
#endif
        if (rank_local) exchange(L, du, -1);
        if (simple_gs || L.part) axpy(n3, (T)1, du, u);
        if (!final_residual && iterations == 0) break;
        if (L.split && !simple_gs && !(level == 0 && !cfg.systemBCProject) && !no_lres) {
            if (plan.path != GsPlan::CHAINED) {
                const bool subtracted = (plan.path == GsPlan::COLOUR || plan.path == GsPlan::PAIR) && !L.part;
                if (!subtracted) HOT_LAUNCH(this, "gs_hdiff", k_gs_hdiff<T>, div_up(n3, 256), 256, 0, n3, hdu, du);
                HOT_LAUNCH(this, lname("gs_residual", L.id).c_str(), (k_gs_residual<T, true>), xcd_grid(div_up(L.n, 4)), 256, 0, L.col.p, L.val.p, L.rowcnt.p, hdu, du, r, L.n, L.mask(),
                    rank_local ? L.owner.p : (const uint8_t*)nullptr, comm.rank, (rank_local && L.l1) ? L.gsE.p : (const T*)nullptr);
            }
            else
                HOT_LAUNCH(this, lname("gs_residual", L.id).c_str(), k_gs_residual<T>, xcd_grid(div_up(L.n, 4)), 256, 0, L.col.p, L.val.p, L.rowcnt.p, hdu, du, r, L.n, L.mask(),
                    rank_local ? L.owner.p : (const uint8_t*)nullptr, comm.rank, (rank_local && L.l1) ? L.gsE.p : (const T*)nullptr);
            if (!hm) exchange(L, r, -1);
        }
        else {
            spmv_dev(L, du, dAu);
            if (level == 0 && !cfg.systemBCProject) project_dev(dAu);
            axpy(n3, (T)-1, dAu, r);
        }
    }
}

template __global__ void k_gs_fill_unset<double>(size_t n, double* x);

template struct Ctx<float>;
template struct Ctx<double>;

}
```

hot_amd/csrc/mg_solve.hip:

```cpp
#include "hot_impl.h"
#include "hot_svd.h"

namespace hot {

template <class T>
__global__ void k_axpy(size_t n, T a, const T* __restrict__ x, T* y)
{
    size_t i = (size_t)blockIdx.x * blockDim.x + threadIdx.x;
    if (i < n) y[i] += a * x[i];
}
template <class T>
__global__ void k_axpy_dev(size_t n, const double* a, double sign, const T* __restrict__ x, T* y)
{
    size_t i = (size_t)blockIdx.x * blockDim.x + threadIdx.x;
    T s = (T)(sign * (*a));
    if (i < n) y[i] += s * x[i];
}
template <class T>
__global__ void k_xpay_dev(size_t n, const double* a, const T* __restrict__ x, T* y)
{
    size_t i = (size_t)blockIdx.x * blockDim.x + threadIdx.x;
    T s = (T)(*a);
    if (i < n) y[i] = x[i] + s * y[i];
}
template <class T>
__global__ __launch_bounds__(256) void k_dot(size_t n, const T* __restrict__ x, const T* __restrict__ y, double* out, GridRed gr, const uint8_t* __restrict__ mask)
{
    __shared__ double red[4];
    double s = 0;
    const size_t stride = (size_t)gridDim.x * 256;
    for (size_t i0 = (size_t)blockIdx.x * 256 + threadIdx.x; i0 < n; i0 += 4 * stride) {
        T xv[4], yv[4];
        bool on[4];
#pragma unroll
        for (int u = 0; u < 4; ++u) {
            const size_t i = i0 + u * stride, ic = i < n ? i : i0;
            on[u] = i < n && (!mask || mask[ic / 3]);
            xv[u] = on[u] ? x[ic] : (T)0, yv[u] = on[u] ? y[ic] : (T)0;
        }
#pragma unroll
        for (int u = 0; u < 4; ++u)
            if (on[u]) s += (double)(xv[u] * yv[u]);
    }
    double t = block_sum_256<double>(s, red);
    grid_sum_store(t, 0.0, 1, gr, out, nullptr, red);
}
template <class T>
void Ctx<T>::axpy(size_t n, T a, const T* x, T* y)
{
    HOT_LAUNCH(this, "axpy", k_axpy<T>, div_up(n, 256), 256, 0, n, a, x, y);
}
template <class T>
void Ctx<T>::axpy_dev(size_t n, const double* a, double sign, const T* x, T* y)
{
    HOT_LAUNCH(this, "axpy", k_axpy_dev<T>, div_up(n, 256), 256, 0, n, a, sign, x, y);
}
template <class T>
__global__ __launch_bounds__(256) void k_copy(size_t n, const T* __restrict__ x, T* __restrict__ y)
{
    for (size_t i = (size_t)blockIdx.x * 256 + threadIdx.x; i < n; i += (size_t)gridDim.x * 256) y[i] = x[i];
}
template <class T>
__global__ __launch_bounds__(256) void k_vcycle_start(size_t n, const T* __restrict__ x, T* __restrict__ y, T* __restrict__ y2, T* __restrict__ z)
{
    for (size_t i = (size_t)blockIdx.x * 256 + threadIdx.x; i < n; i += (size_t)gridDim.x * 256) {
        const T v = x[i];
        y[i] = v, z[i] = (T)0;
        if (y2) y2[i] = v;
    }
}
template <class A, class B>
__global__ __launch_bounds__(256) void k_mg32_convert(size_t n, const A* __restrict__ x, B* __restrict__ y)
{
    for (size_t i = (size_t)blockIdx.x * 256 + threadIdx.x; i < n; i += (size_t)gridDim.x * 256) y[i] = (B)x[i];
}
__global__ __launch_bounds__(256) void k_mg32_absmax(size_t n, const double* __restrict__ x, GridRed gr, double* sc, double* mirror)
{
    __shared__ double red[4];
    __shared__ int s_last;
    const int lane = threadIdx.x & 63, w = threadIdx.x >> 6;
    auto block_max = [&](double m) {
        for (int o = 32; o > 0; o >>= 1) m = fmax(m, __shfl_xor(m, o));
        if (lane == 0) red[w] = m;
        __syncthreads();
        const double r = fmax(fmax(red[0], red[1]), fmax(red[2], red[3]));
        __syncthreads();
        return r;
    };
    double m = 0;
    for (size_t i = (size_t)blockIdx.x * 256 + threadIdx.x; i < n; i += (size_t)gridDim.x * 256) m = fmax(m, fabs(x[i]));
    m = block_max(m);
    const unsigned nb = gridDim.x;
    if (threadIdx.x == 0) {
        __hip_atomic_store(gr.part + blockIdx.x, m, __ATOMIC_RELAXED, __HIP_MEMORY_SCOPE_AGENT);
        asm volatile("s_waitcnt vmcnt(0)" ::: "memory");
        const unsigned prev = __hip_atomic_fetch_add(gr.count, 1u, __ATOMIC_RELAXED, __HIP_MEMORY_SCOPE_AGENT);
        s_last = prev == nb - 1u;
    }
    __syncthreads();
    if (!s_last) return;
    double a = 0;
    for (unsigned i = threadIdx.x; i < nb; i += 256) a = fmax(a, __hip_atomic_load(gr.part + i, __ATOMIC_RELAXED, __HIP_MEMORY_SCOPE_AGENT));
    a = block_max(a);
    if (threadIdx.x == 0) {
        int e = (a > 0.0 && a < (double)INFINITY) ? ilogb(a) : 0;
        e = e < -1022 ? -1022 : e;
        const double down = scalbn(1.0, -e), up = scalbn(1.0, e);
        sc[0] = down, sc[1] = a == 0.0 ? 0.0 : up;
        if (mirror) *mirror = up;
        __hip_atomic_store(gr.count, 0u, __ATOMIC_RELAXED, __HIP_MEMORY_SCOPE_AGENT);
    }
}
__global__ __launch_bounds__(256) void k_mg32_enter(size_t n, const double* __restrict__ x, const double* __restrict__ sc, float* __restrict__ y, float* __restrict__ y2, float* __restrict__ z)
{
    const double down = sc[0];
    for (size_t i = (size_t)blockIdx.x * 256 + threadIdx.x; i < n; i += (size_t)gridDim.x * 256) {
        const float v = (float)(x[i] * down);
        y[i] = v, z[i] = 0.0f;
        if (y2) y2[i] = v;
    }
}
__global__ __launch_bounds__(256) void k_mg32_exit(size_t n, const float* __restrict__ z, const double* __restrict__ sc, double* __restrict__ out)
{
    const double up = sc[1];
    for (size_t i = (size_t)blockIdx.x * 256 + threadIdx.x; i < n; i += (size_t)gridDim.x * 256) out[i] = up == 0.0 ? 0.0 : (double)z[i] * up;
}
template <class T>
void Ctx<T>::widen_dev(size_t n, const float* x, double* y)
{
    if (n) HOT_LAUNCH(this, "mg32_convert", (k_mg32_convert<float, double>), (int)std::min<size_t>(div_up(n, 256), 4096), 256, 0, n, x, y);
}
template <class T>
void Ctx<T>::narrow_dev(size_t n, const double* x, float* y)
{
    if (n) HOT_LAUNCH(this, "mg32_convert", (k_mg32_convert<double, float>), (int)std::min<size_t>(div_up(n, 256), 4096), 256, 0, n, x, y);
}
template <class T>
void Ctx<T>::vcycle_mixed(const T* in, T* out)
{
    if constexpr (sizeof(T) == 8) {
        const size_t n0 = 3 * (size_t)mg32->levels[0]->n;
        double* sc = dscal.p + 230;
        const int grid = std::min(div_up(n0, 1024), 256);
        HOT_LAUNCH(this, "mg32_enter", k_mg32_absmax, grid, 256, 0, n0, in, gred(grid), sc, hscal + 252);
        mg32->mg32_io[0].reserve(n0);
        float* out32 = mg32->mg32_io[0].p;
        mg32->vcycle_head = [this, in, sc, n0](float* y, float* y2, float* z) {
            HOT_LAUNCH(this, "mg32_enter", k_mg32_enter, (int)std::min<size_t>(div_up(n0, 256), 2048), 256, 0, n0, in, sc, y, y2, z);
        };
        struct Unhook {
            Ctx<float>* c;
            ~Unhook() { c->vcycle_head = nullptr; }
        } unhook{ mg32 };
        mg32->vcycle_dev(nullptr, out32);
        fold_shadow_stats();
        HOT_LAUNCH(this, "mg32_exit", k_mg32_exit, (int)std::min<size_t>(div_up(n0, 256), 2048), 256, 0, n0, out32, sc, out);
    }
}

template <class T>
void Ctx<T>::copy(size_t n, const T* x, T* y)
{
    if (n) HOT_LAUNCH(this, "copy", k_copy<T>, (int)std::min<size_t>(div_up(n, 256), 2048), 256, 0, n, x, y);
}
template <class T>
void Ctx<T>::zero(size_t n, T* y)
{
    HOT_HIP(hipMemsetAsync(y, 0, n * sizeof(T), stream));
}
template <class T>
void Ctx<T>::dot_to(size_t n, const T* x, const T* y, double* out, double* mirror)
{
    const int grid = std::min(div_up(n, 1024), 256);
    if (vmask) {
        HOT_LAUNCH(this, "dot", k_dot<T>, grid, 256, 0, n, x, y, out, gred(grid), vmask);
        reduce_scalars(out, 1);
        if (mirror) HOT_HIP(hipMemcpyAsync(mirror, out, sizeof(double), hipMemcpyDeviceToHost, stream));
        return;
    }
    HOT_LAUNCH(this, "dot", k_dot<T>, grid, 256, 0, n, x, y, out, gred(grid, mirror), (const uint8_t*)nullptr);
}
template <class T>
double Ctx<T>::dot_host(size_t n, const T* x, const T* y)
{
    const int grid = std::min(div_up(n, 1024), 256);
    HOT_LAUNCH(this, "dot", k_dot<T>, grid, 256, 0, n, x, y, dscal.p + 100, gred(grid, hscal + 100, true), vmask);
    wait_ticket();
    if (vmask) c_allreduce(hscal + 100, 1, HOT_COMM_F64, HOT_COMM_SUM, false);
    return hscal[100];
}

template <class T>
__global__ __launch_bounds__(256) void k_spmv(const int32_t* __restrict__ col, const T* __restrict__ val, const T* __restrict__ x, T* __restrict__ y, int n, const uint8_t* __restrict__ own)
{
    const int lane = threadIdx.x & 63;
    const int row = xcd_block() * 4 + (threadIdx.x >> 6);
    if (row >= n || (own && !own[row])) return;
    const int32_t* c = col + (int64_t)row * 125;
    const T* v = val + (int64_t)row * 1125;
    T s0 = 0, s1 = 0, s2 = 0;
#pragma unroll
    for (int r = 0; r < 2; ++r) {
        int k = lane + 64 * r;
        if (k < 125) {
            int j = c[k];
            const T* b = v + k * 9;
            T x0 = x[3 * (int64_t)j], x1 = x[3 * (int64_t)j + 1], x2 = x[3 * (int64_t)j + 2];
            s0 += b[0] * x0 + b[3] * x1 + b[6] * x2;
            s1 += b[1] * x0 + b[4] * x1 + b[7] * x2;
            s2 += b[2] * x0 + b[5] * x1 + b[8] * x2;
        }
    }
    s0 = wave_sum(s0), s1 = wave_sum(s1), s2 = wave_sum(s2);
    if (lane == 0) y[3 * (int64_t)row] = s0, y[3 * (int64_t)row + 1] = s1, y[3 * (int64_t)row + 2] = s2;
}
template <class T>
__global__ __launch_bounds__(256) void k_apmv_sub(const int32_t* __restrict__ apc, const T* __restrict__ apv, const T* __restrict__ e, T* __restrict__ r, int n, const uint8_t* __restrict__ own,
    T* unset )
{
    const int lane = threadIdx.x & 63;
    const int row = xcd_block() * 4 + (threadIdx.x >> 6);
    if (row >= n) return;
    if (unset && lane < 3) gs_store_unset(unset + 3 * (int64_t)row + lane);
    if (own && !own[row]) return;
    const int j = nt_load(apc + (int64_t)row * 64 + lane);
    const int slot = __popcll(__ballot(j >= 0) & ((1ull << lane) - 1ull));
    T s0 = (T)0, s1 = (T)0, s2 = (T)0;
    if (j >= 0) {
        const T* bp = apv + ((int64_t)row * 64 + slot) * 9;
        T b[9];
#pragma unroll
        for (int t = 0; t < 9; ++t) b[t] = nt_load(bp + t);
        const T x0 = e[3 * (int64_t)j], x1 = e[3 * (int64_t)j + 1], x2 = e[3 * (int64_t)j + 2];
        s0 = b[0] * x0 + b[3] * x1 + b[6] * x2;
        s1 = b[1] * x0 + b[4] * x1 + b[7] * x2;
        s2 = b[2] * x0 + b[5] * x1 + b[8] * x2;
    }
    s0 = wave_sum(s0), s1 = wave_sum(s1), s2 = wave_sum(s2);
    if (lane == 0) r[3 * (int64_t)row] -= s0, r[3 * (int64_t)row + 1] -= s1, r[3 * (int64_t)row + 2] -= s2;
}
__device__ __forceinline__ bool cg_active(double zTr, double tol) { return !(zTr < tol); }
template <class T>
__global__ void k_cg_setup(double* s, double* hm)
{
    const double tol = (double)(T)(s[7] * 0.25);
    s[8] = tol;
    s[1] = s[2] = s[3] = s[4] = s[5] = s[6] = s[9] = 0.0;
    hm[0] = s[0], hm[1] = 0.0, hm[2] = tol;
}
template <class T>
__global__ __launch_bounds__(256) void k_cg_spmv_dot(const int32_t* __restrict__ col, const T* __restrict__ val, const T* __restrict__ du, T* __restrict__ dAu, int n, double* s, GridRed gr)
{
    __shared__ double red[4];
    const bool roll = s[6] != 0.0;
    const double cur = roll ? s[4] : s[0];
    if (blockIdx.x == 0 && threadIdx.x == 0 && roll) s[0] = s[4];
    if (!cg_active(cur, s[8])) return;
    const int lane = threadIdx.x & 63;
    const int row = blockIdx.x * 4 + (threadIdx.x >> 6);
    double part = 0;
    if (row < n) {
        const int32_t* c = col + (int64_t)row * 125;
        const T* v = val + (int64_t)row * 1125;
        T s0 = 0, s1 = 0, s2 = 0;
#pragma unroll
        for (int r = 0; r < 2; ++r) {
            int k = lane + 64 * r;
            if (k < 125) {
                int j = c[k];
                const T* b = v + k * 9;
                T x0 = du[3 * (int64_t)j], x1 = du[3 * (int64_t)j + 1], x2 = du[3 * (int64_t)j + 2];
                s0 += b[0] * x0 + b[3] * x1 + b[6] * x2;
                s1 += b[1] * x0 + b[4] * x1 + b[7] * x2;
                s2 += b[2] * x0 + b[5] * x1 + b[8] * x2;
            }
        }
        s0 = wave_sum(s0), s1 = wave_sum(s1), s2 = wave_sum(s2);
        if (lane == 0) {
            dAu[3 * (int64_t)row] = s0, dAu[3 * (int64_t)row + 1] = s1, dAu[3 * (int64_t)row + 2] = s2;
            part = (double)(s0 * du[3 * (int64_t)row]) + (double)(s1 * du[3 * (int64_t)row + 1]) + (double)(s2 * du[3 * (int64_t)row + 2]);
        }
    }
    if (lane == 0) red[threadIdx.x >> 6] = part;
    __syncthreads();
    const double t = threadIdx.x == 0 ? red[0] + red[1] + red[2] + red[3] : 0.0;
    __syncthreads();
    grid_sum_store(t, 0.0, 1, gr, s + 1, nullptr, red);
}
template <class T>
__global__ __launch_bounds__(256) void k_cg_update(const T* __restrict__ Dinv, const T* __restrict__ du, const T* __restrict__ dAu, T* __restrict__ u, T* __restrict__ r, T* __restrict__ z, int n, double* s, GridRed gr)
{
    __shared__ double red[4];
    const int i = blockIdx.x * 256 + threadIdx.x;
    if (!cg_active(s[0], s[8])) return;
    const double omega = s[0] / s[1];
    const T wp = (T)omega, wm = (T)(-omega);
    double part = 0;
    if (i < n) {
        T rr[3];
#pragma unroll
        for (int c = 0; c < 3; ++c) {
            u[3 * (int64_t)i + c] += wp * du[3 * (int64_t)i + c];
            rr[c] = r[3 * (int64_t)i + c] + wm * dAu[3 * (int64_t)i + c];
            r[3 * (int64_t)i + c] = rr[c];
        }
        const T* d = Dinv + 9 * (int64_t)i;
        const T z0 = d[0] * rr[0] + d[3] * rr[1] + d[6] * rr[2], z1 = d[1] * rr[0] + d[4] * rr[1] + d[7] * rr[2], z2 = d[2] * rr[0] + d[5] * rr[1] + d[8] * rr[2];
        z[3 * (int64_t)i] = z0, z[3 * (int64_t)i + 1] = z1, z[3 * (int64_t)i + 2] = z2;
        part = (double)(z0 * rr[0]) + (double)(z1 * rr[1]) + (double)(z2 * rr[2]);
    }
    const double t = block_sum_256<double>(part, red);
    grid_sum_store(t, 0.0, 1, gr, s + 4, nullptr, red);
}
template <class T>
__global__ void k_cg_direction(size_t n3, const T* __restrict__ z, T* __restrict__ du, double* s, double* hm, double* ticket, double ticket_val)
{
    const size_t i = (size_t)blockIdx.x * blockDim.x + threadIdx.x;
    const bool act = cg_active(s[0], s[8]);
    if (act && i < n3) du[i] = z[i] + (T)(s[4] / s[0]) * du[i];
    if (i == 0) {
        if (act) {
            s[6] = 1.0;
            const double cnt = s[9] + 1.0;
            s[9] = cnt;
            hm[0] = s[4], hm[1] = cnt;
        }
        if (ticket) host_ticket_store(ticket, ticket_val);
    }
}
template <class T, int RPW = 0>
__global__ __launch_bounds__(1024) void k_cg_persist(const int32_t* __restrict__ col, const T* __restrict__ val, const T* __restrict__ Dinv, const T* __restrict__ init, T* __restrict__ u,
    T* __restrict__ r, T* __restrict__ z, T* du, T* __restrict__ dAu, int n, int max_iters, unsigned phase0 , double* dep , int SS , double* hm, double* ticket, double ticket_val,
    int* err )
{
    __shared__ double red[32], sres[2];
    __shared__ int s_bail;
    enum { CG_DI = 0, CG_U = 9, CG_R = 12, CG_Z = 15, CG_D = 18, CG_AD = 21 };
    __shared__ T cg_row[RPW > 0 ? 16 : 1][RPW > 0 ? RPW : 1][24];
    const int tid = threadIdx.x, lane = tid & 63, w = __builtin_amdgcn_readfirstlane(tid >> 6);
    const int G = gridDim.x, wg = blockIdx.x;
    unsigned phase = phase0;
    if (tid == 0) s_bail = 0;
    auto ldu = [&](int64_t j, int c) { return __hip_atomic_load(du + 3 * j + c, __ATOMIC_RELAXED, __HIP_MEMORY_SCOPE_AGENT); };
    auto sdu = [&](int64_t j, int c, T v) { __hip_atomic_store(du + 3 * j + c, v, __ATOMIC_RELAXED, __HIP_MEMORY_SCOPE_AGENT); };
    auto all_sum = [&](double v0, double v1, double& o0, double& o1) -> bool {
        asm volatile("s_waitcnt vmcnt(0)" ::: "memory");
        if (lane == 0) red[w] = v0, red[16 + w] = v1;
        __syncthreads();
        double* d = dep + (size_t)(phase & 3u) * G * SS;
        if (tid == 0) {
            double t0 = 0, t1 = 0;
            for (int k = 0; k < 16; ++k) t0 += red[k], t1 += red[16 + k];
            double* dn = dep + (size_t)((phase + 2u) & 3u) * G * SS + (size_t)wg * SS;
            __hip_atomic_store((unsigned long long*)dn, GsUnset<double>::bits, __ATOMIC_RELAXED, __HIP_MEMORY_SCOPE_AGENT);
            __hip_atomic_store((unsigned long long*)(dn + 1), GsUnset<double>::bits, __ATOMIC_RELAXED, __HIP_MEMORY_SCOPE_AGENT);
            __hip_atomic_store(d + (size_t)wg * SS, t0, __ATOMIC_RELAXED, __HIP_MEMORY_SCOPE_AGENT);
            __hip_atomic_store(d + (size_t)wg * SS + 1, t1, __ATOMIC_RELAXED, __HIP_MEMORY_SCOPE_AGENT);
        }
        if (w < 2) {
            const double* dv = d + w;
            double a = 0;
            int spins = 0, bail = 0;
            for (;;) {
                bool all = true;
                a = 0;
                for (int k = lane; k < G; k += 64) {
                    const double x = __hip_atomic_load(dv + (size_t)k * SS, __ATOMIC_RELAXED, __HIP_MEMORY_SCOPE_AGENT);
                    all = all && !GsUnset<double>::is(x);
                    a += x;
                }
                if (__all(all)) break;
                __builtin_amdgcn_s_sleep(1);
                if (++spins > (1 << 21) || ((spins & 255) == 0 && *(volatile int*)err)) {
                    *(volatile int*)err = 1;
                    bail = 1;
                    break;
                }
            }
            a = wave_sum(a);
            if (lane == 0) {
                sres[w] = a;
                if (bail) s_bail = 1;
            }
        }
        __syncthreads();
        if (s_bail) return false;
        o0 = wave_first(sres[0]), o1 = wave_first(sres[1]);
        ++phase;
        return true;
    };
    auto scale = [&](int64_t i, const T (&v)[3], T (&o)[3]) {
        const T* d = Dinv + 9 * i;
        o[0] = d[0] * v[0] + d[3] * v[1] + d[6] * v[2], o[1] = d[1] * v[0] + d[4] * v[1] + d[7] * v[2], o[2] = d[2] * v[0] + d[5] * v[1] + d[8] * v[2];
    };
    const int stride = 16 * G;
    if constexpr (RPW > 0) {
        int rowq[RPW];
        int32_t mc[RPW][2];
        T mv[RPW][2][9];
        double p0 = 0, p1 = 0;
#pragma unroll
        for (int q = 0; q < RPW; ++q) {
            const int row = wg * 16 + w + q * stride;
            rowq[q] = row < n ? row : -1;
            const int64_t rc = row < n ? row : 0;
#pragma unroll
            for (int h = 0; h < 2; ++h) {
                const int k = min(lane + 64 * h, 124);
                mc[q][h] = col[rc * 125 + k];
#pragma unroll
                for (int e = 0; e < 9; ++e) mv[q][h][e] = (lane + 64 * h < 125) ? val[rc * 1125 + k * 9 + e] : (T)0;
            }
            if (lane == 0) {
                T* st = cg_row[w][q];
                T di[9], a[3], za[3], rr[3], zz[3];
#pragma unroll
                for (int e = 0; e < 9; ++e) di[e] = Dinv[9 * rc + e], st[CG_DI + e] = di[e];
#pragma unroll
                for (int c = 0; c < 3; ++c) a[c] = init[3 * rc + c], rr[c] = r[3 * rc + c], st[CG_U + c] = u[3 * rc + c], st[CG_AD + c] = (T)0;
#pragma unroll
                for (int c = 0; c < 3; ++c) za[c] = di[c] * a[0] + di[3 + c] * a[1] + di[6 + c] * a[2], zz[c] = di[c] * rr[0] + di[3 + c] * rr[1] + di[6 + c] * rr[2];
                if (rowq[q] >= 0) {
                    p0 += (double)(za[0] * a[0]) + (double)(za[1] * a[1]) + (double)(za[2] * a[2]);
                    p1 += (double)(zz[0] * rr[0]) + (double)(zz[1] * rr[1]) + (double)(zz[2] * rr[2]);
                    for (int c = 0; c < 3; ++c) sdu(row, c, zz[c]);
                }
#pragma unroll
                for (int c = 0; c < 3; ++c) st[CG_R + c] = rr[c], st[CG_Z + c] = zz[c], st[CG_D + c] = zz[c];
            }
        }
        double zTr0, zTr;
        if (!all_sum(p0, p1, zTr0, zTr)) return;
        const double tol = (double)(T)(zTr0 * 0.25);
        extern __shared__ double cg_lds[];
        T* ldsdu = (T*)cg_lds;
        const int n3 = 3 * n;
        auto pull_du = [&]() {
            const int n16 = n3 >> 1;
            for (int e0 = 0; e0 < n16; e0 += 4 * 1024) {
                double2 v[4];
#pragma unroll
                for (int k = 0; k < 4; ++k) {
                    const unsigned eb = 16u * (unsigned)min(e0 + k * 1024 + tid, n16 - 1);
                    asm volatile("global_load_dwordx4 %0, %1, %2 sc0 sc1" : "=v"(v[k]) : "v"(eb), "s"(du) : "memory");
                }
                asm volatile("s_waitcnt vmcnt(0)" ::: "memory");
#pragma unroll
                for (int k = 0; k < 4; ++k) {
                    const int e = e0 + k * 1024 + tid;
                    if (e < n16) ((double2*)ldsdu)[e] = v[k];
                }
            }
            if ((n3 & 1) && tid == 0) ldsdu[n3 - 1] = ldu(n - 1, 2);
            __syncthreads();
        };
        int cnt = 0;
#ifdef HOT_AB_KERNELS
        unsigned long long tk[8] = { 0, 0, 0, 0, 0, 0, 0, 0 }, t0_ = wall_clock64();
#define CG_TK(i) \
    do { \
        const unsigned long long t_ = wall_clock64(); \
        tk[i] += t_ - t0_, t0_ = t_; \
    } while (0)
#else
#define CG_TK(i)
#endif
        for (; cnt < max_iters && cg_active(zTr, tol); ++cnt) {
            pull_du();
            CG_TK(0);
            double pd = 0;
#pragma unroll
            for (int q = 0; q < RPW; ++q) {
                T s0 = 0, s1 = 0, s2 = 0;
#pragma unroll
                for (int h = 0; h < 2; ++h) {
                    if (lane + 64 * h < 125) {
                        const int j = mc[q][h];
                        const T* b = mv[q][h];
                        const T x0 = ldsdu[3 * j], x1 = ldsdu[3 * j + 1], x2 = ldsdu[3 * j + 2];
                        s0 += b[0] * x0 + b[3] * x1 + b[6] * x2;
                        s1 += b[1] * x0 + b[4] * x1 + b[7] * x2;
                        s2 += b[2] * x0 + b[5] * x1 + b[8] * x2;
                    }
                }
                s0 = wave_sum(s0), s1 = wave_sum(s1), s2 = wave_sum(s2);
                if (lane == 0) {
                    T* st = cg_row[w][q];
                    st[CG_AD] = s0, st[CG_AD + 1] = s1, st[CG_AD + 2] = s2;
                    if (rowq[q] >= 0) pd += (double)(s0 * st[CG_D]) + (double)(s1 * st[CG_D + 1]) + (double)(s2 * st[CG_D + 2]);
                }
            }
            CG_TK(1);
            double dAd, unused;
            if (!all_sum(pd, 0.0, dAd, unused)) return;
            CG_TK(2);
            const double omega = zTr / dAd;
            const T wp = (T)omega, wm = (T)(-omega);
            double pz = 0;
            if (lane == 0) {
#pragma unroll
                for (int q = 0; q < RPW; ++q) {
                    T* st = cg_row[w][q];
                    T rr[3], zz[3];
#pragma unroll
                    for (int c = 0; c < 3; ++c) st[CG_U + c] += wp * st[CG_D + c], rr[c] = st[CG_R + c] + wm * st[CG_AD + c];
#pragma unroll
                    for (int c = 0; c < 3; ++c) zz[c] = st[CG_DI + c] * rr[0] + st[CG_DI + 3 + c] * rr[1] + st[CG_DI + 6 + c] * rr[2];
                    if (rowq[q] >= 0) pz += (double)(zz[0] * rr[0]) + (double)(zz[1] * rr[1]) + (double)(zz[2] * rr[2]);
#pragma unroll
                    for (int c = 0; c < 3; ++c) st[CG_R + c] = rr[c], st[CG_Z + c] = zz[c];
                }
            }
            CG_TK(3);
            double zTrNew;
            if (!all_sum(pz, 0.0, zTrNew, unused)) return;
            CG_TK(4);
            const T beta = (T)(zTrNew / zTr);
            if (lane == 0) {
#pragma unroll
                for (int q = 0; q < RPW; ++q) {
                    T* st = cg_row[w][q];
                    T dd[3];
#pragma unroll
                    for (int c = 0; c < 3; ++c) dd[c] = st[CG_Z + c] + beta * st[CG_D + c], st[CG_D + c] = dd[c];
                    if (rowq[q] >= 0)
                        for (int c = 0; c < 3; ++c) sdu(rowq[q], c, dd[c]);
                }
            }
            zTr = zTrNew;
            CG_TK(5);
            if (!all_sum(0.0, 0.0, unused, unused)) return;
            CG_TK(6);
        }
#ifdef HOT_AB_KERNELS
        if (tid == 0 && wg == 0)
            for (int i = 0; i < 7; ++i) hm[8 + i] = (double)tk[i];
#endif
#pragma unroll
        for (int q = 0; q < RPW; ++q)
            if (lane == 0 && rowq[q] >= 0) {
                const T* st = cg_row[w][q];
                for (int c = 0; c < 3; ++c) {
                    const int64_t e = 3 * (int64_t)rowq[q] + c;
                    u[e] = st[CG_U + c], r[e] = st[CG_R + c], z[e] = st[CG_Z + c], dAu[e] = st[CG_AD + c];
                }
            }
        if (tid == 0 && wg == 0) {
            hm[0] = zTr, hm[1] = (double)cnt, hm[2] = tol, hm[3] = (double)(phase & 3u);
            if (ticket) host_ticket_store(ticket, ticket_val);
        }
        return;
    }
    double p0 = 0, p1 = 0;
    for (int row = wg * 16 + w; row < n; row += stride) {
        if (lane == 0) {
            T a[3] = { init[3 * (int64_t)row], init[3 * (int64_t)row + 1], init[3 * (int64_t)row + 2] }, za[3];
            scale(row, a, za);
            p0 += (double)(za[0] * a[0]) + (double)(za[1] * a[1]) + (double)(za[2] * a[2]);
            T b[3] = { r[3 * (int64_t)row], r[3 * (int64_t)row + 1], r[3 * (int64_t)row + 2] }, zb[3];
            scale(row, b, zb);
            for (int c = 0; c < 3; ++c) z[3 * (int64_t)row + c] = zb[c], sdu(row, c, zb[c]);
            p1 += (double)(zb[0] * b[0]) + (double)(zb[1] * b[1]) + (double)(zb[2] * b[2]);
        }
    }
    double zTr0, zTr;
    if (!all_sum(p0, p1, zTr0, zTr)) return;
    const double tol = (double)(T)(zTr0 * 0.25);
    int cnt = 0;
    for (; cnt < max_iters && cg_active(zTr, tol); ++cnt) {
        double pd = 0;
        for (int row = wg * 16 + w; row < n; row += stride) {
            const int32_t* c = col + (int64_t)row * 125;
            const T* v = val + (int64_t)row * 1125;
            T s0 = 0, s1 = 0, s2 = 0;
#pragma unroll
            for (int q = 0; q < 2; ++q) {
                const int k = lane + 64 * q;
                if (k < 125) {
                    const int64_t j = c[k];
                    const T* b = v + k * 9;
                    const T x0 = ldu(j, 0), x1 = ldu(j, 1), x2 = ldu(j, 2);
                    s0 += b[0] * x0 + b[3] * x1 + b[6] * x2;
                    s1 += b[1] * x0 + b[4] * x1 + b[7] * x2;
                    s2 += b[2] * x0 + b[5] * x1 + b[8] * x2;
                }
            }
            s0 = wave_sum(s0), s1 = wave_sum(s1), s2 = wave_sum(s2);
            if (lane == 0) {
                dAu[3 * (int64_t)row] = s0, dAu[3 * (int64_t)row + 1] = s1, dAu[3 * (int64_t)row + 2] = s2;
                pd += (double)(s0 * ldu(row, 0)) + (double)(s1 * ldu(row, 1)) + (double)(s2 * ldu(row, 2));
            }
        }
        double dAd, unused;
        if (!all_sum(pd, 0.0, dAd, unused)) return;
        const double omega = zTr / dAd;
        const T wp = (T)omega, wm = (T)(-omega);
        double pz = 0;
        for (int row = wg * 16 + w; row < n; row += stride) {
            if (lane == 0) {
                T rr[3], zz[3];
                for (int c = 0; c < 3; ++c) {
                    u[3 * (int64_t)row + c] += wp * ldu(row, c);
                    rr[c] = r[3 * (int64_t)row + c] + wm * dAu[3 * (int64_t)row + c];
                    r[3 * (int64_t)row + c] = rr[c];
                }
                scale(row, rr, zz);
                for (int c = 0; c < 3; ++c) z[3 * (int64_t)row + c] = zz[c];
                pz += (double)(zz[0] * rr[0]) + (double)(zz[1] * rr[1]) + (double)(zz[2] * rr[2]);
            }
        }
        double zTrNew;
        if (!all_sum(pz, 0.0, zTrNew, unused)) return;
        const T beta = (T)(zTrNew / zTr);
        for (int row = wg * 16 + w; row < n; row += stride)
            if (lane == 0)
                for (int c = 0; c < 3; ++c) sdu(row, c, z[3 * (int64_t)row + c] + beta * ldu(row, c));
        zTr = zTrNew;
        if (!all_sum(0.0, 0.0, unused, unused)) return;
    }
    if (tid == 0) {
        if (wg == 0) {
            hm[0] = zTr, hm[1] = (double)cnt, hm[2] = tol, hm[3] = (double)(phase & 3u);
            if (ticket) host_ticket_store(ticket, ticket_val);
        }
    }
}

template <class T>
__global__ void k_scal_v(size_t n, T a, T* x)
{
    size_t i = (size_t)blockIdx.x * blockDim.x + threadIdx.x;
    if (i < n) x[i] *= a;
}
template <class T>
void Ctx<T>::scal(size_t n, T a, T* x)
{
    HOT_LAUNCH(this, "scal", k_scal_v<T>, div_up(n, 256), 256, 0, n, a, x);
}
template <class T>
void Ctx<T>::spmv_dev(Level<T>& L, const T* x, T* y)
{
    if (L.part && halo_mode()) halo_gather(L, const_cast<T*>(x));
    HOT_LAUNCH(this, lname("spmv", L.id).c_str(), k_spmv<T>, xcd_grid(div_up(L.n, 4)), 256, 0, L.col.p, L.val.p, x, y, L.n, L.mask());
    if (!halo_mode()) exchange(L, y, -1);
}

template <class T>
__global__ void k_restrict(const int32_t* __restrict__ child, const T* __restrict__ fine, T* coarse, int nc, const uint8_t* __restrict__ coarse_own, const uint8_t* __restrict__ fine_own,
    T* unset , T* zero_out = nullptr )
{
    int e = blockIdx.x * blockDim.x + threadIdx.x;
    if (e >= 3 * nc) return;
    if (unset) gs_store_unset(unset + e);
    if (zero_out) zero_out[e] = (T)0;
    int I = e / 3, d = e - 3 * I;
    if (coarse_own && !coarse_own[I]) return;
    int ci[27];
#pragma unroll
    for (int q = 0; q < 27; ++q) ci[q] = child[I * 27 + q];
    T fv[27];
#pragma unroll
    for (int q = 0; q < 27; ++q) fv[q] = fine[3 * (int64_t)(ci[q] < 0 ? 0 : ci[q]) + d];
    T s = 0;
#pragma unroll
    for (int q = 0; q < 27; ++q) {
        const T w = ((q / 9 != 1) ? (T)0.5 : (T)1) * (((q / 3) % 3 != 1) ? (T)0.5 : (T)1) * ((q % 3 != 1) ? (T)0.5 : (T)1);
        s = (ci[q] < 0 || (fine_own && !fine_own[ci[q]])) ? s : s + w * fv[q];
    }
    coarse[e] = s;
}
template <class T>
__global__ void k_prolong(const int32_t* __restrict__ pcol, const T* __restrict__ pw, const T* __restrict__ coarse, T* fine, int n, const uint8_t* __restrict__ own)
{
    int e = blockIdx.x * blockDim.x + threadIdx.x;
    if (e >= 3 * n) return;
    int i = e / 3, d = e - 3 * i;
    if (own && !own[i]) return;
    T s = 0;
    for (int l = 0; l < 8; ++l) s += pw[8 * (int64_t)i + l] * coarse[3 * (int64_t)pcol[8 * (int64_t)i + l] + d];
    fine[e] = s;
}
template <class T>
int Ctx<T>::smoother_kind(int level, bool top) const
{
    const bool baseline = cfg.useBaselineMultigrid != 0;
    const int splitLevel = cfg.topDownMGS ? 1 : cfg.levelCnt - 1;
    return (level < splitLevel && !top) ? (baseline ? 5 : cfg.smoother) : (baseline ? 2 : cfg.coarseSolver);
}
template <class T>
bool Ctx<T>::gs_marks_wanted(int level) const
{
    return smoother_kind(level) == 5 && gs_plan(*levels[level]).marks;
}
template <class T>
void Ctx<T>::restrict_dev(int level, const T* fine, T* coarse, T* zero_coarse)
{
    Level<T>& C = *levels[level + 1];
    Level<T>& F = *levels[level];
    if (F.part && halo_mode()) {
        if (zero_coarse) zero(3 * (size_t)C.n, zero_coarse);
        if (C.part) {
            halo_gather(F, const_cast<T*>(fine));
            HOT_LAUNCH(this, "restrict", k_restrict<T>, div_up(3 * (size_t)C.n, 256), 256, 0, C.child.p, fine, coarse, C.n, C.own.p, (const uint8_t*)nullptr, (T*)nullptr);
        }
        else {
            HOT_LAUNCH(this, "restrict", k_restrict<T>, div_up(3 * (size_t)C.n, 256), 256, 0, C.child.p, fine, coarse, C.n, (const uint8_t*)nullptr, F.own.p, (T*)nullptr);
            CommTag tag(this, "coarse_vector_allreduce");
            c_allreduce(coarse, 3 * (int64_t)C.n, REAL, HOT_COMM_SUM, true);
        }
        return;
    }
    T* mark = gs_marks_wanted(level + 1) ? C.tmp.p : (T*)nullptr;
    HOT_LAUNCH(this, "restrict", k_restrict<T>, div_up(3 * (size_t)C.n, 256), 256, 0, C.child.p, fine, coarse, C.n, (const uint8_t*)nullptr, (const uint8_t*)nullptr, mark, zero_coarse);
    unset_level = mark ? level + 1 : -1;
}
template <class T>
void Ctx<T>::prolong_dev(int level, const T* coarse, T* fine)
{
    Level<T>& F = *levels[level];
    Level<T>& C = *levels[level + 1];
    const bool hm = F.part && halo_mode();
    if (hm && C.part) halo_gather(C, const_cast<T*>(coarse));
    HOT_LAUNCH(this, "prolong", k_prolong<T>, div_up(3 * (size_t)F.n, 256), 256, 0, F.pcol.p, F.pw.p, coarse, fine, F.n, hm ? F.own.p : (const uint8_t*)nullptr);
}

template <class T>
__global__ void k_scale(const T* __restrict__ D, const T* __restrict__ r, T* mr, int n)
{
    int i = blockIdx.x * blockDim.x + threadIdx.x;
    if (i >= n) return;
    const T* d = D + 9 * (int64_t)i;
    T a = r[3 * (int64_t)i], b = r[3 * (int64_t)i + 1], c = r[3 * (int64_t)i + 2];
    mr[3 * (int64_t)i] = d[0] * a + d[3] * b + d[6] * c;
    mr[3 * (int64_t)i + 1] = d[1] * a + d[4] * b + d[7] * c;
    mr[3 * (int64_t)i + 2] = d[2] * a + d[5] * b + d[8] * c;
}

template <class T>
__global__ void k_cheb_start(T* v, size_t n3)
{
    size_t e = (size_t)blockIdx.x * blockDim.x + threadIdx.x;
    if (e < n3) v[e] = ((((unsigned)e * 2654435761u) >> 16) & 1u) ? (T)1 : (T)-1;
}
template <class T>
__global__ void k_abs(T* v, size_t n3)
{
    size_t e = (size_t)blockIdx.x * blockDim.x + threadIdx.x;
    if (e < n3) v[e] = v[e] < 0 ? -v[e] : v[e];
}
template <class T>
__global__ void k_div1(T* v, T c, size_t n3)
{
    size_t e = (size_t)blockIdx.x * blockDim.x + threadIdx.x;
    if (e < n3) v[e] = v[e] / c;
}
template <class T>
void Ctx<T>::estimate_2norm(Level<T>& L, double tol)
{
    MaskScope mscope(this, halo_mode() ? L.mask() : nullptr);
    constexpr int MaxIters = 512;
    size_t n3 = 3 * (size_t)L.n;
    T *v = L.du.p, *x = L.dAu.p;
    HOT_LAUNCH(this, "cheb_start", k_cheb_start<T>, div_up(n3, 256), 256, 0, v, n3);
    spmv_dev(L, v, x);
    HOT_LAUNCH(this, "cheb_abs", k_abs<T>, div_up(n3, 256), 256, 0, x, n3);
    T e = (T)std::sqrt(dot_host(n3, x, x));
    if (e == 0) {
        L.lMin = L.lMax = 0;
        return;
    }
    HOT_LAUNCH(this, "cheb_div", k_div1<T>, div_up(n3, 256), 256, 0, x, e, n3);
    T e0 = 0;
    for (int iter = 0; iter < MaxIters && std::abs(e - e0) > (T)tol * e; ++iter) {
        e0 = e;
        spmv_dev(L, x, v);
        spmv_dev(L, v, x);
        T normx = (T)std::sqrt(dot_host(n3, x, x));
        e = normx / (T)std::sqrt(dot_host(n3, v, v));
        HOT_LAUNCH(this, "cheb_div", k_div1<T>, div_up(n3, 256), 256, 0, x, normx, n3);
    }
    L.lMax = e;
    L.lMin = L.lMax / 30;
}

template <class T>
void Ctx<T>::block_apply_dev(const T* D, const T* in, T* out, int n)
{
    HOT_LAUNCH(this, "diag_scale", k_scale<T>, div_up(n, 256), 256, 0, D, in, out, n);
}
template <class T>
void Ctx<T>::scale_dev(Level<T>& L, const T* in, T* out)
{
    HOT_LAUNCH(this, "diag_scale", k_scale<T>, div_up(L.n, 256), 256, 0, L.diagInv.p, in, out, L.n);
}

template <class T>
__global__ void k_cg_scalars(double* s, int what)
{
    if (what == 0) {
        s[2] = s[0] / s[1];
        s[3] = -s[2];
    }
    else {
        s[5] = s[4] / s[0];
        s[0] = s[4];
    }
}

template <class T>
void Ctx<T>::smooth_dev(int level, int kind, int iterations, T tolerance, T* u, T* r, T* du, T* dAu, bool final_residual)
{
    Level<T>& L = *levels[level];
    size_t n3 = 3 * (size_t)L.n;
    MaskScope mscope(this, halo_mode() ? L.mask() : nullptr);
    const bool tmp_marked = unset_level == level;
    unset_level = -1;
    auto Aproject = [&](T* v) {
        if (level == 0 && !cfg.systemBCProject) project_dev(v);
    };
    auto scaler = [&](const T* in, T* out) { scale_dev(L, in, out); };
    if (kind == 0) {
        for (; iterations--;) {
            scaler(r, du);
            scal(n3, (T)cfg.topomega, du);
            axpy(n3, (T)1, du, u);
            if (!final_residual && iterations == 0) break;
            spmv_dev(L, du, dAu);
            Aproject(dAu);
            axpy(n3, (T)-1, dAu, r);
        }
    }
    else if (kind == 1) {
        for (; iterations--;) {
            double rr = dot_host(n3, r, r);
            if (std::sqrt(rr) * (in_scale_h ? *in_scale_h : 1.0) < (double)tolerance) break;
            scaler(r, du);
            spmv_dev(L, du, dAu);
            Aproject(dAu);
            double a = dot_host(n3, du, r), b = dot_host(n3, du, dAu);
            T omega = (T)(a / b);
            axpy(n3, omega, du, u);
            axpy(n3, -omega, dAu, r);
        }
    }
    else if (kind == 2) {
        T* z = L.tmp.p;
        double* s = dscal.p + 40;
        const bool cg_unfused = ab_flag("HOT_CG_UNFUSED");
        const bool fused = !cg_unfused && !(level == 0 && !cfg.systemBCProject) && !L.part;
        int cnt = 0;
        double zTrk = 0, tol = 0;
        if (fused && sizeof(T) == 8 && L.n <= 65536 && !gs_no_chain && !sharded() && !ab_flag("HOT_CG_LAUNCHES")) {
            const int G = std::min(std::min(ab_int("HOT_CG_WGS", 256), device_cus()), div_up(L.n, 16));
            const int cg_ss = ab_int("HOT_CG_SLOT_STRIDE", 32);
            if (!cg_dep.p || cg_bar_dirty || cg_G != G) {
                cg_dep.reserve((size_t)4 * 256 * cg_ss);
                HOT_LAUNCH(this, "gs_fill_unset", k_gs_fill_unset<double>, div_up((size_t)4 * 256 * cg_ss, 256), 256, 0, (size_t)4 * 256 * cg_ss, cg_dep.p);
                cg_bar_dirty = false, cg_G = G, cg_phase = 0;
            }
            const bool cg_resident = L.n <= 2 * 16 * G && 3 * (size_t)L.n * sizeof(double) <= 150 * 1024 && !ab_flag("HOT_CG_STREAM");
            if (cg_resident && !attr_cg_set) {
                HOT_HIP(hipFuncSetAttribute((const void*)k_cg_persist<T, 2>, hipFuncAttributeMaxDynamicSharedMemorySize, 150 * 1024));
                attr_cg_set = true;
            }
            if (cg_resident)
                HOT_LAUNCH(this, lname("cg_persistent", L.id).c_str(), (k_cg_persist<T, 2>), G, 1024, 3 * (size_t)L.n * sizeof(double), L.col.p, L.val.p, L.diagInv.p, L.initialResidual.p, u, r, z, du, dAu, L.n, iterations, cg_phase, cg_dep.p, cg_ss,
                    hscal + 40, hscal + 251, new_ticket(), (int*)(hscal + 250));
            else
                HOT_LAUNCH(this, lname("cg_persistent", L.id).c_str(), k_cg_persist<T>, G, 1024, 0, L.col.p, L.val.p, L.diagInv.p, L.initialResidual.p, u, r, z, du, dAu, L.n, iterations, cg_phase, cg_dep.p, cg_ss,
                    hscal + 40, hscal + 251, new_ticket(), (int*)(hscal + 250));
            wait_ticket();
            cnt = (int)hscal[41];
            if (ab_flag("HOT_CG_DBG"))
                fprintf(stderr, "cg_persistent level %d: %d rows, %d workgroups, %d iterations; ticks pull %.0f product %.0f barrier1 %.0f update %.0f barrier2 %.0f direction %.0f barrier3 %.0f\n", L.id, L.n, G, cnt,
                    hscal[48], hscal[49], hscal[50], hscal[51], hscal[52], hscal[53], hscal[54]);
            cg_phase = (cg_phase + 1u + 3u * (unsigned)cnt) & 3u;
            HOT_CHECK((unsigned)hscal[43] == cg_phase, HOT_ERR_DEVICE, "k_cg_persist passed another number of barriers than the host counts: the next launch would start on the wrong set of deposit slots");
            iterations = 0;
        }
        else if (fused) {
            scaler(L.initialResidual.p, z);
            dot_to(n3, z, L.initialResidual.p, s + 7);
            scaler(r, z);
            copy(n3, z, du);
            dot_to(n3, z, r, s);
            HOT_LAUNCH(this, "cg_setup", k_cg_setup<T>, 1, 1, 0, s, hscal + 40);
            int group = std::max(1, std::min(cg_group, 16));
            bool active = true;
            while (iterations > 0 && active) {
                const int g = std::min(group, iterations);
                for (int k = 0; k < g; ++k) {
                    HOT_LAUNCH(this, lname("spmv", L.id).c_str(), k_cg_spmv_dot<T>, div_up(L.n, 4), 256, 0, L.col.p, L.val.p, du, dAu, L.n, s, gred(div_up(L.n, 4)));
                    HOT_LAUNCH(this, "cg_update", k_cg_update<T>, div_up(L.n, 256), 256, 0, L.diagInv.p, du, dAu, u, r, z, L.n, s, gred(div_up(L.n, 256)));
                    const bool last = k + 1 == g;
                    HOT_LAUNCH(this, "cg_direction", k_cg_direction<T>, div_up(n3, 256), 256, 0, n3, z, du, s, hscal + 40, last ? hscal + 251 : (double*)nullptr, last ? new_ticket() : 0.0);
                }
                iterations -= g;
                wait_ticket();
                active = !(hscal[40] < hscal[42]);
                group = 2;
            }
            cnt = (int)hscal[41];
            cg_group = cnt;
            iterations = 0;
        }
        else {
            scaler(L.initialResidual.p, z);
            double zTrk0 = dot_host(n3, z, L.initialResidual.p);
            scaler(r, z);
            copy(n3, z, du);
            zTrk = dot_host(n3, z, r);
            tol = (double)(T)(zTrk0 * 0.25);
            HOT_HIP(hipMemcpyAsync(s, &zTrk, sizeof(double), hipMemcpyHostToDevice, stream));
        }
        for (; iterations-- > 0;) {
            if (zTrk < tol) break;
            spmv_dev(L, du, dAu);
            Aproject(dAu);
            dot_to(n3, dAu, du, s + 1);
            HOT_LAUNCH(this, "cg_scalars", k_cg_scalars<T>, 1, 1, 0, s, 0);
            axpy_dev(n3, s + 2, 1.0, du, u);
            axpy_dev(n3, s + 3, 1.0, dAu, r);
            scaler(r, z);
            dot_to(n3, z, r, s + 4);
            HOT_LAUNCH(this, "cg_scalars", k_cg_scalars<T>, 1, 1, 0, s, 1);
            HOT_LAUNCH(this, "xpay", k_xpay_dev<T>, div_up(n3, 256), 256, 0, n3, s + 5, z, du);
            HOT_HIP(hipMemcpyAsync(hscal + 40, s, sizeof(double), hipMemcpyDeviceToHost, stream));
            sync();
            zTrk = hscal[40];
            ++cnt;
        }
        stats.linear_iterations += cnt;
    }
    else if (kind == 6) {
        T* p = L.tmp.p;
        T d = (T)((L.lMax + L.lMin) / 2), c = (T)((L.lMax - L.lMin) / 2);
        int cnt = 1;
        iterations--;
        scaler(r, p);
        T alpha = 1 / d, beta;
        copy(n3, p, du);
        spmv_dev(L, du, dAu);
        Aproject(dAu);
        axpy(n3, alpha, du, u);
        axpy(n3, -alpha, dAu, r);
        for (; iterations-- > 0; ++cnt) {
            scaler(r, p);
            beta = (T)0.5 * c * c * alpha * alpha;
            if (cnt > 1) beta *= (T)0.5;
            alpha = 1 / (d - beta / alpha);
            scal(n3, beta, du);
            axpy(n3, (T)1, p, du);
            spmv_dev(L, du, dAu);
            Aproject(dAu);
            axpy(n3, alpha, du, u);
            if (!final_residual && iterations <= 0) break;
            axpy(n3, -alpha, dAu, r);
        }
    }
    else if (kind == 7)
        ic_smooth_dev(L, u, r, dAu);
    else if (kind == 5)
        gs_smooth_dev(level, iterations, u, r, du, dAu, final_residual, tmp_marked);
    else
        HOT_CHECK(false, HOT_ERR_INVALID, "unsupported smoother kind");
}

template <class T>
void Ctx<T>::vcycle_dev(const T* in, T* out)
{
    if (mixed()) {
        vcycle_mixed(in, out);
        return;
    }
    int levelCnt = (int)levels.size();
    int times = cfg.times, levelscale = cfg.levelscale;
    int splitLevel;
    auto downIter = [&](int level) { return times + level * levelscale; };
    auto upIter = [&](int level) { return cfg.topDownMGS ? 0 : times + level * levelscale; };
    const bool baseline = cfg.useBaselineMultigrid != 0;
    auto topIter = [&](int level) {
        if (cfg.topDownMGS || baseline) return 10000;
        if (cfg.levelCnt == 1) return times + level * levelscale;
        if (!(cfg.coarseSolver == 2 || cfg.coarseSolver == 6)) return (times + level * levelscale) * 3;
        return 10000;
    };
    splitLevel = cfg.topDownMGS ? 1 : cfg.levelCnt - 1;
    T tolTop = (T)(cfg.cneps * cfg.cneps);
    auto run = [&](bool regular, int level, T* sol, int its, bool final_residual = true) {
        Level<T>& L = *levels[level];
        smooth_dev(level, smoother_kind(level, !regular), its, regular ? (T)0 : tolTop, sol, L.residual.p, L.du.p, L.dAu.p, final_residual);
    };
    stats.vcycles++;
    Level<T>& L0 = *levels[0];
    size_t n0 = 3 * (size_t)L0.n;
    if (vcycle_head)
        vcycle_head(L0.residual.p, levelCnt > 1 ? (T*)nullptr : L0.initialResidual.p, out);
    else
    HOT_LAUNCH(this, "vcycle_start", k_vcycle_start<T>, (int)std::min<size_t>(div_up(n0, 256), 2048), 256, 0, n0, in, L0.residual.p, levelCnt > 1 ? (T*)nullptr : L0.initialResidual.p, out);

    if (levelCnt > 1) restrict_dev(0, L0.residual.p, levels[1]->initialResidual.p);
    for (int l = 1; l < levelCnt - 1; ++l) restrict_dev(l, levels[l]->initialResidual.p, levels[l + 1]->initialResidual.p);
    int level;
    for (level = 0; level < levelCnt - 1; ++level) {
        T* sol = level == 0 ? out : levels[level]->sol.p;
        run(level < splitLevel, level, sol, level < splitLevel ? upIter(level) : topIter(level));
        restrict_dev(level, levels[level]->residual.p, levels[level + 1]->residual.p, levels[level + 1]->sol.p);
    }
    run(false, level, level == 0 ? out : levels[level]->sol.p, topIter(level));
    for (--level; level >= 0; --level) {
        Level<T>& L = *levels[level];
        T* sol = level == 0 ? out : L.sol.p;
        size_t n3 = 3 * (size_t)L.n;
        prolong_dev(level, levels[level + 1]->sol.p, L.du.p);
        axpy(n3, (T)1, L.du.p, sol);
        const bool full_spmv = ab_flag("HOT_MG_FULL_SPMV");
        if (full_spmv) {
            spmv_dev(L, L.du.p, L.dAu.p);
            axpy(n3, (T)-1, L.dAu.p, L.residual.p);
        }
        else
        {
            T* mark = gs_marks_wanted(level) ? L.tmp.p : (T*)nullptr;
            HOT_LAUNCH(this, lname("apmv", L.id).c_str(), k_apmv_sub<T>, xcd_grid(div_up(L.n, 4)), 256, 0, L.apc.p, L.apv.p, levels[level + 1]->sol.p, L.residual.p, L.n, L.mask(), mark);
            unset_level = mark ? level : -1;
        }
        if (L.part && !halo_mode() && smoother_kind(level) != 5)
            exchange(L, L.residual.p, -1);
        run(level < splitLevel, level, sol, level < splitLevel ? downIter(level) : topIter(level), false);
    }
}

template <class T>
void Ctx<T>::precondition_dev(const T* in, T* out)
{
    HOT_CHECK(mixed() || (!levels.empty() && levels[0]->built), HOT_ERR_INVALID, "preconditioner used before hot_build_mg");
    vcycle_dev(in, out);
}

template <class T>
void Ctx<T>::spmv(int32_t level, const void* x, void* y)
{
    if constexpr (sizeof(T) == 8)
        if (mixed() && level >= 1) {
            need(level < nlevels(), "level out of range");
            Level<float>& S = *mg32->levels[level];
            mixed_apply(x, 3 * (size_t)S.n, y, 3 * (size_t)S.n, [&](float* a, float* b) { mg32->spmv_dev(S, a, b); });
            return;
        }
    need(level >= 0 && level < (int)levels.size(), "level out of range");
    Level<T>& L = *levels[level];
    size_t n3 = 3 * (size_t)L.n;
    DBuf<T> a, b;
    a.reserve(n3), b.reserve(n3);
    HOT_HIP(hipMemcpyAsync(a.p, x, n3 * sizeof(T), hipMemcpyDefault, stream));
    spmv_dev(L, a.p, b.p);
    if (halo_mode()) gather_all(L, b.p);
    download(y, b.p, n3);
    sync();
}
template <class T>
void Ctx<T>::restrict_(int32_t level, const void* fine, void* coarse)
{
    if constexpr (sizeof(T) == 8)
        if (mixed()) {
            need(level >= 0 && level + 1 < nlevels(), "level out of range");
            mixed_apply(fine, 3 * (size_t)mg32->levels[level]->n, coarse, 3 * (size_t)mg32->levels[level + 1]->n, [&](float* a, float* b) { mg32->restrict_dev(level, a, b), mg32->unset_level = -1; });
            return;
        }
    need(level >= 0 && level + 1 < (int)levels.size(), "level out of range");
    size_t nf = 3 * (size_t)levels[level]->n, nc = 3 * (size_t)levels[level + 1]->n;
    DBuf<T> a, b;
    a.reserve(nf), b.reserve(nc);
    HOT_HIP(hipMemcpyAsync(a.p, fine, nf * sizeof(T), hipMemcpyDefault, stream));
    restrict_dev(level, a.p, b.p);
    if (halo_mode()) gather_all(*levels[level + 1], b.p);
    download(coarse, b.p, nc);
    sync();
}
template <class T>
void Ctx<T>::prolong(int32_t level, const void* coarse, void* fine)
{
    if constexpr (sizeof(T) == 8)
        if (mixed()) {
            need(level >= 0 && level + 1 < nlevels(), "level out of range");
            mixed_apply(coarse, 3 * (size_t)mg32->levels[level + 1]->n, fine, 3 * (size_t)mg32->levels[level]->n, [&](float* a, float* b) { mg32->prolong_dev(level, a, b); });
            return;
        }
    need(level >= 0 && level + 1 < (int)levels.size(), "level out of range");
    size_t nf = 3 * (size_t)levels[level]->n, nc = 3 * (size_t)levels[level + 1]->n;
    DBuf<T> a, b;
    a.reserve(nc), b.reserve(nf);
    HOT_HIP(hipMemcpyAsync(a.p, coarse, nc * sizeof(T), hipMemcpyDefault, stream));
    prolong_dev(level, a.p, b.p);
    if (halo_mode()) gather_all(*levels[level], b.p);
    download(fine, b.p, nf);
    sync();
}
template <class T>
void Ctx<T>::smooth(int32_t level, int32_t kind, int32_t iterations, double tol, void* u, void* r, const void* r0)
{
    if constexpr (sizeof(T) == 8)
        if (mixed()) {
            need(level >= 0 && level < nlevels() && mg32->levels[level]->built, "hot_smooth: level not built (hot_build_mg)");
            Level<float>& S = *mg32->levels[level];
            const size_t n3 = 3 * (size_t)S.n;
            DBuf<T> keep[3];
            for (auto& k : keep) k.reserve(n3);
            HOT_HIP(hipMemcpyAsync(keep[0].p, u, n3 * sizeof(T), hipMemcpyDefault, stream));
            HOT_HIP(hipMemcpyAsync(keep[1].p, r, n3 * sizeof(T), hipMemcpyDefault, stream));
            HOT_HIP(hipMemcpyAsync(keep[2].p, r0 ? r0 : r, n3 * sizeof(T), hipMemcpyDefault, stream));
            for (auto& b : mg32->mg32_io) b.reserve(n3);
            hscal[252] = 1.0;
            with_gs_retry([&] {
                narrow_dev(n3, keep[0].p, mg32->mg32_io[0].p), narrow_dev(n3, keep[1].p, mg32->mg32_io[1].p), narrow_dev(n3, keep[2].p, S.initialResidual.p);
                mg32->smooth_dev(level, kind, iterations, (float)tol, mg32->mg32_io[0].p, mg32->mg32_io[1].p, S.du.p, S.dAu.p);
                fold_shadow_stats();
                sync();
            });
            widen_dev(n3, mg32->mg32_io[0].p, keep[0].p), widen_dev(n3, mg32->mg32_io[1].p, keep[1].p);
            download(u, keep[0].p, n3);
            download(r, keep[1].p, n3);
            sync();
            return;
        }
    need(level >= 0 && level < (int)levels.size() && levels[level]->built, "hot_smooth: level not built (hot_build_mg)");
    Level<T>& L = *levels[level];
    size_t n3 = 3 * (size_t)L.n;
    DBuf<T> du_, dr_, r0_;
    du_.reserve(n3), dr_.reserve(n3), r0_.reserve(n3);
    HOT_HIP(hipMemcpyAsync(r0_.p, r0 ? r0 : r, n3 * sizeof(T), hipMemcpyDefault, stream));
    with_gs_retry([&] {
        HOT_HIP(hipMemcpyAsync(du_.p, u, n3 * sizeof(T), hipMemcpyDefault, stream));
        HOT_HIP(hipMemcpyAsync(dr_.p, r, n3 * sizeof(T), hipMemcpyDefault, stream));
        HOT_HIP(hipMemcpyAsync(L.initialResidual.p, r0_.p, n3 * sizeof(T), hipMemcpyDeviceToDevice, stream));
        smooth_dev(level, kind, iterations, (T)tol, du_.p, dr_.p, L.du.p, L.dAu.p);
        if (halo_mode()) gather_all(L, du_.p), gather_all(L, dr_.p);
        sync();
    });
    download(u, du_.p, n3);
    download(r, dr_.p, n3);
    sync();
}
template <class T>
void Ctx<T>::vcycle(const void* in, void* out)
{
    need(mixed() || (!levels.empty() && levels[0]->built), "hot_vcycle before hot_build_mg");
    size_t n3 = 3 * (size_t)Nn;
    HOT_HIP(hipMemcpyAsync(work0.p, in, n3 * sizeof(T), hipMemcpyDefault, stream));
    with_gs_retry([&] {
        vcycle_dev(work0.p, work1.p);
        if (halo_mode()) gather_all(*levels[0], work1.p);
        sync();
    });
    download(out, work1.p, n3);
    sync();
}

template struct Ctx<float>;
template struct Ctx<double>;

}
```

Baseline: 3.028 ms/iter.

## Chain forward and backward Gauss-Seidel half-sweeps into one symmetric persistent launch

```diff
diff --git a/hot_amd/csrc/gs_sweep_body.h b/hot_amd/csrc/gs_sweep_body.h
--- /dev/null
+++ b/hot_amd/csrc/gs_sweep_body.h
@@ -0,0 +1,291 @@
+    extern __shared__ __attribute__((aligned(16))) char gs_smem[];
+    constexpr int TRI = GsLds<T, SB>::TRI;
+    static_assert(!WINV || SB == 64, "the inverse images are whole-block images");
+#ifdef HOT_GS_CLOCKS
+    unsigned long long gclk_[5] = { 0, 0, 0, 0, 0 }, gt0_ = clock64();
+#endif
+    constexpr int RQ = 4, NW = SB / RQ;
+    auto ld3 = [&](int64_t j, T& x0, T& x1, T& x2) {
+        x0 = __hip_atomic_load(x + 3 * j, __ATOMIC_RELAXED, __HIP_MEMORY_SCOPE_AGENT), x1 = __hip_atomic_load(x + 3 * j + 1, __ATOMIC_RELAXED, __HIP_MEMORY_SCOPE_AGENT),
+        x2 = __hip_atomic_load(x + 3 * j + 2, __ATOMIC_RELAXED, __HIP_MEMORY_SCOPE_AGENT);
+        int spins = 0;
+        while (GsUnset<T>::is(x0) || GsUnset<T>::is(x1) || GsUnset<T>::is(x2)) {
+            __builtin_amdgcn_s_sleep(2);
+            if (++spins > (1 << 21) || ((spins & 1023) == 0 && *(volatile int*)err)) {
+                *(volatile int*)err = 1;
+                break;
+            }
+            x0 = __hip_atomic_load(x + 3 * j, __ATOMIC_RELAXED, __HIP_MEMORY_SCOPE_AGENT), x1 = __hip_atomic_load(x + 3 * j + 1, __ATOMIC_RELAXED, __HIP_MEMORY_SCOPE_AGENT),
+            x2 = __hip_atomic_load(x + 3 * j + 2, __ATOMIC_RELAXED, __HIP_MEMORY_SCOPE_AGENT);
+        }
+    };
+    T* tri = (T*)gs_smem;
+    T* sv = tri + (WINV ? GsWinv<T>::img_elems : 9 * TRI);
+    int32_t* nodes = (int32_t*)(sv + 3 * SB);
+    const int tid = threadIdx.x, lane = tid & 63, w = tid >> 6;
+    const int b = P.block0[p] + ((int)blockIdx.x - P.wg_begin[p]);
+    const int lo = P.sub[p] * SB;
+    const int start = block_start[b] + lo, cnt = max(0, min(SB, block_start[b + 1] - start));
+    int32_t* rng = nodes + SB;
+    T* sDinv = (T*)(nodes + 5 * SB);
+    T* sD = sDinv + 9 * SB;
+    T* srhs = sD + 9 * SB;
+    if (!WINV)
+        for (int e = tid; e < 9 * TRI; e += 64 * NW) tri[e] = (T)0;
+    if (tid < SB) nodes[tid] = tid < cnt ? gs_order[start + tid] : -1;
+    __syncthreads();
+    GS_CLK(0);
+    if (WINV) {
+        constexpr int IMG_BYTES = GsWinv<T>::img_elems * (int)sizeof(T);
+        const char* wg = (const char*)(gs_w + ((size_t)b * 2 + (DFWD ? 0 : 1)) * GsWinv<T>::img_elems);
+        for (int c = w; c * 1024 < IMG_BYTES; c += NW) {
+            const int off = c * 1024 + lane * 16;
+            if (off < IMG_BYTES)
+                __builtin_amdgcn_global_load_lds((const __attribute__((address_space(1))) void*)(wg + off), (__attribute__((address_space(3))) void*)((char*)tri + c * 1024), 16, 0, 0);
+        }
+    }
+    for (int e = tid; e < 9 * cnt; e += 64 * NW) {
+        const int64_t i = nodes[e / 9];
+        sDinv[e] = diagBlockInv[9 * i + e % 9];
+        if (DFWD) sD[e] = diagVal[9 * i + e % 9];
+    }
+    if constexpr (SYM && !DFWD) {
+        for (int e = tid; e < 3 * cnt; e += 64 * NW) {
+            const T* src = rhs + 3 * (int64_t)nodes[e / 3] + e % 3;
+            T v = __hip_atomic_load(src, __ATOMIC_RELAXED, __HIP_MEMORY_SCOPE_AGENT);
+            int spins = 0;
+            while (GsUnset<T>::is(v)) {
+                __builtin_amdgcn_s_sleep(2);
+                if (++spins > (1 << 21) || ((spins & 1023) == 0 && *(volatile int*)err)) {
+                    *(volatile int*)err = 1;
+                    break;
+                }
+                v = __hip_atomic_load(src, __ATOMIC_RELAXED, __HIP_MEMORY_SCOPE_AGENT);
+            }
+            srhs[e] = v;
+        }
+    }
+    else
+        for (int e = tid; e < 3 * cnt; e += 64 * NW) srhs[e] = rhs[3 * (int64_t)nodes[e / 3] + e % 3];
+    if (unset_next)
+        for (int e = tid; e < 3 * cnt; e += 64 * NW) gs_store_unset(unset_next + 3 * (int64_t)nodes[e / 3] + e % 3);
+    T bv[RQ][9];
+    int jj[RQ], node[RQ], kb2[RQ], ke[RQ];
+    const bool same_dir = SYM ? (p > 0 && ((P.color[p - 1] ^ P.color[p]) & GS_PASS_BWD) == 0) : p > 0;
+    const bool first_sub = !same_dir || P.color[p - 1] != P.color[p];
+    const bool head = DFWD ? first_sub : !first_sub;
+    bool late[RQ];
+    const uint32_t prevkey = same_dir ? ((uint32_t)(SYM ? P.color[p - 1] & 7 : P.color[p - 1]) << 8) | (uint32_t)P.sub[p - 1] : 0xffffffffu;
+    if constexpr (WINV) {
+        int4 rc[RQ];
+#pragma unroll
+        for (int q = 0; q < RQ; ++q) {
+            const int ii = w + NW * q;
+            jj[q] = -1, kb2[q] = 0, ke[q] = 0, late[q] = false;
+            node[q] = ii < cnt ? __builtin_amdgcn_readfirstlane(nodes[ii]) : -1;
+#pragma unroll
+            for (int e = 0; e < 9; ++e) bv[q][e] = (T)0;
+        }
+#pragma unroll
+        for (int q = 0; q < RQ; ++q) rc[q] = node[q] >= 0 ? *(const int4*)(rowcnt + 4 * (int64_t)node[q]) : make_int4(0, 0, 0, 0);
+#pragma unroll
+        for (int q = 0; q < RQ; ++q) {
+            if (node[q] < 0) continue;
+            const int64_t i = node[q];
+            const int kbeg = DFWD ? 0 : rc[q].x + rc[q].y + 1 + rc[q].z, kend = DFWD ? rc[q].x : kbeg + rc[q].w;
+            kb2[q] = head ? kbeg + 64 : kbeg, ke[q] = head ? kend : kend - 64;
+            const int k = head ? kbeg + lane : kend - 64 + lane;
+            if (k >= kbeg && k < kend) {
+                jj[q] = col[i * 125 + k];
+                const T* bb = val + (i * 125 + k) * 9;
+#pragma unroll
+                for (int e = 0; e < 9; ++e) bv[q][e] = bb[e];
+            }
+        }
+#pragma unroll
+        for (int q = 0; q < RQ; ++q)
+            if (jj[q] >= 0) {
+                const uint32_t keyj = ckey[jj[q]];
+                late[q] = (((keyj >> 28) << 8) | (((keyj & 127u) - 1u) / (uint32_t)SB)) == prevkey;
+            }
+    }
+    else
+#pragma unroll
+    for (int q = 0; q < RQ; ++q) {
+        const int ii = w + NW * q;
+        jj[q] = -1, node[q] = -1, kb2[q] = 0, ke[q] = 0, late[q] = false;
+#pragma unroll
+        for (int e = 0; e < 9; ++e) bv[q][e] = (T)0;
+        if (ii < cnt) {
+            const int i = nodes[ii];
+            node[q] = i;
+            const int po = rowcnt[4 * i], pi = rowcnt[4 * i + 1], fi = rowcnt[4 * i + 2], fo = rowcnt[4 * i + 3];
+            const int kbeg = DFWD ? 0 : po + pi + 1, kend = DFWD ? po + pi : po + pi + 1 + fi + fo;
+            const int ibeg = DFWD ? po : kbeg, iend = DFWD ? po + pi : kbeg + fi;
+            kb2[q] = head ? kbeg + 64 : kbeg, ke[q] = head ? kend : kend - 64;
+            rng[ii] = kb2[q], rng[SB + ii] = ke[q];
+            const int k = head ? kbeg + lane : kend - 64 + lane;
+            if (k >= kbeg && k < kend) {
+                const int j = col[(int64_t)i * 125 + k];
+                const T* bb = val + ((int64_t)i * 125 + k) * 9;
+#pragma unroll
+                for (int e = 0; e < 9; ++e) bv[q][e] = bb[e];
+                jj[q] = j;
+                const uint32_t keyj = ckey[j];
+                late[q] = (((keyj >> 28) << 8) | (((keyj & 127u) - 1u) / (uint32_t)SB)) == prevkey;
+                if (k >= ibeg && k < iend) {
+                    const int l = (int)(keyj & 127u) - 1 - lo;
+                    if (l >= 0 && l < SB) {
+                        if (!WINV) {
+                            const int idx = DFWD ? gs_tri_fwd<SB>(ii, l) : gs_tri_bwd(ii, l);
+                            gs_store_tri<T>(tri, TRI, idx, diagBlockInv + 9 * (int64_t)i, bv[q]);
+                        }
+                        jj[q] = -1;
+                    }
+                }
+            }
+        }
+    }
+    __syncthreads();
+    GS_CLK(1);
+    auto is_late = [&](uint32_t keyj) { return (((keyj >> 28) << 8) | (((keyj & 127u) - 1u) / (uint32_t)SB)) == prevkey; };
+    bool tail_late[RQ];
+#pragma unroll
+    for (int q = 0; q < RQ; ++q) {
+        const int ii = w + NW * q;
+        tail_late[q] = false;
+        if (ii >= cnt) continue;
+        const int i = WINV ? node[q] : nodes[ii], kt0 = WINV ? kb2[q] : rng[ii], kt1 = WINV ? ke[q] : rng[SB + ii];
+        T e0 = 0, e1 = 0, e2 = 0;
+        if (jj[q] >= 0 && !late[q]) {
+            const int64_t j = jj[q];
+            T x0, x1, x2;
+            ld3(j, x0, x1, x2);
+            e0 = bv[q][0] * x0 + bv[q][3] * x1 + bv[q][6] * x2;
+            e1 = bv[q][1] * x0 + bv[q][4] * x1 + bv[q][7] * x2;
+            e2 = bv[q][2] * x0 + bv[q][5] * x1 + bv[q][8] * x2;
+        }
+        bool tl = false;
+        for (int k = kt0 + lane; k < kt1; k += 64) {
+            const int j = col[(int64_t)i * 125 + k];
+            const T* bb = val + ((int64_t)i * 125 + k) * 9;
+            const uint32_t keyj = ckey[j], keyi = ckey[i];
+            const int l = (int)(keyj & 127u) - 1 - lo;
+            if ((keyj >> 7) == (keyi >> 7) && l >= 0 && l < SB) {
+                if (!WINV) {
+                    const int idx = DFWD ? gs_tri_fwd<SB>(ii, l) : gs_tri_bwd(ii, l);
+                    T bt[9];
+#pragma unroll
+                    for (int e = 0; e < 9; ++e) bt[e] = bb[e];
+                    gs_store_tri<T>(tri, TRI, idx, diagBlockInv + 9 * (int64_t)i, bt);
+                }
+            }
+            else if (is_late(keyj))
+                tl = true;
+            else {
+                T x0, x1, x2;
+                ld3(j, x0, x1, x2);
+                e0 += bb[0] * x0 + bb[3] * x1 + bb[6] * x2;
+                e1 += bb[1] * x0 + bb[4] * x1 + bb[7] * x2;
+                e2 += bb[2] * x0 + bb[5] * x1 + bb[8] * x2;
+            }
+        }
+        tail_late[q] = __ballot(tl) != 0ull;
+        e0 = wave_sum(e0), e1 = wave_sum(e1), e2 = wave_sum(e2);
+        if (lane == 0) srhs[3 * ii] -= e0, srhs[3 * ii + 1] -= e1, srhs[3 * ii + 2] -= e2;
+    }
+    GS_CLK(2);
+    const T* val_again = val;
+    asm volatile("" : "+s"(val_again));
+#pragma unroll
+    for (int q = 0; q < RQ; ++q) {
+        const int ii = w + NW * q;
+        if (ii >= cnt) continue;
+        const int i = WINV ? node[q] : nodes[ii], kt0 = WINV ? kb2[q] : rng[ii], kt1 = WINV ? ke[q] : rng[SB + ii];
+        T s0 = 0, s1 = 0, s2 = 0;
+        if (jj[q] >= 0 && late[q]) {
+            const int64_t j = jj[q];
+            const T* bb = val_again + ((int64_t)i * 125 + (head ? kt0 - 64 : kt1) + lane) * 9;
+            T bl[9];
+#pragma unroll
+            for (int e = 0; e < 9; ++e) bl[e] = bb[e];
+            T x0, x1, x2;
+            ld3(j, x0, x1, x2);
+            s0 = bl[0] * x0 + bl[3] * x1 + bl[6] * x2;
+            s1 = bl[1] * x0 + bl[4] * x1 + bl[7] * x2;
+            s2 = bl[2] * x0 + bl[5] * x1 + bl[8] * x2;
+        }
+        if (tail_late[q]) {
+            for (int k = kt0 + lane; k < kt1; k += 64) {
+                const int j = col[(int64_t)i * 125 + k];
+                const T* bb = val + ((int64_t)i * 125 + k) * 9;
+                const uint32_t keyj = ckey[j], keyi = ckey[i];
+                const int l = (int)(keyj & 127u) - 1 - lo;
+                if (!((keyj >> 7) == (keyi >> 7) && l >= 0 && l < SB) && is_late(keyj)) {
+                    T x0, x1, x2;
+                    ld3(j, x0, x1, x2);
+                    s0 += bb[0] * x0 + bb[3] * x1 + bb[6] * x2;
+                    s1 += bb[1] * x0 + bb[4] * x1 + bb[7] * x2;
+                    s2 += bb[2] * x0 + bb[5] * x1 + bb[8] * x2;
+                }
+            }
+        }
+        s0 = wave_sum(s0), s1 = wave_sum(s1), s2 = wave_sum(s2);
+        if (lane == 0) gs_store_rhs<T>(sv, ii, sDinv + 9 * ii, srhs[3 * ii] - s0, srhs[3 * ii + 1] - s1, srhs[3 * ii + 2] - s2);
+    }
+    __syncthreads();
+    GS_CLK(3);
+#ifdef HOT_GS_CLOCKS
+#define GS_CLK_OUT() \
+    do { \
+        GS_CLK(4); \
+        if (tid == 0) \
+            for (int i = 0; i < 5; ++i) atomicAdd(&gs_clk[p * 8 + i], gclk_[i]); \
+        if (tid == 0) atomicAdd(&gs_clk[p * 8 + 7], 1ull); \
+    } while (0)
+#else
+#define GS_CLK_OUT()
+#endif
+    if (WINV) {
+        const bool cin = lane < cnt;
+        const T ac0 = cin ? sv[3 * lane] : (T)0, ac1 = cin ? sv[3 * lane + 1] : (T)0, ac2 = cin ? sv[3 * lane + 2] : (T)0;
+        T h0 = 0, h1 = 0, h2 = 0;
+#pragma unroll
+        for (int k = 0; k < 4; ++k) {
+            const int rr = 4 * w + k;
+            if (rr >= cnt) break;
+            const bool act = DFWD ? lane < rr : (lane > rr && cin);
+            const int idx = act ? gs_winv_idx<DFWD>(rr, lane) : TRI - 1;
+            T Lw[9];
+#pragma unroll
+            for (int e = 0; e < 9; ++e) Lw[e] = tri[e * TRI + idx];
+            T t0 = Lw[0] * ac0 + Lw[3] * ac1 + Lw[6] * ac2, t1 = Lw[1] * ac0 + Lw[4] * ac1 + Lw[7] * ac2, t2 = Lw[2] * ac0 + Lw[5] * ac1 + Lw[8] * ac2;
+            t0 = wave_sum(t0), t1 = wave_sum(t1), t2 = wave_sum(t2);
+            if (lane == k) h0 = sv[3 * rr] + t0, h1 = sv[3 * rr + 1] + t1, h2 = sv[3 * rr + 2] + t2;
+        }
+        const int me = 4 * w + lane;
+        if (lane < 4 && me < cnt) {
+            const int64_t i = nodes[me];
+            __hip_atomic_store(x + 3 * i, h0, __ATOMIC_RELAXED, __HIP_MEMORY_SCOPE_AGENT);
+            __hip_atomic_store(x + 3 * i + 1, h1, __ATOMIC_RELAXED, __HIP_MEMORY_SCOPE_AGENT);
+            __hip_atomic_store(x + 3 * i + 2, h2, __ATOMIC_RELAXED, __HIP_MEMORY_SCOPE_AGENT);
+            if (DFWD) {
+                const T* dd = sD + 9 * me;
+                const T d0 = dd[0] * h0 + dd[3] * h1 + dd[6] * h2, d1 = dd[1] * h0 + dd[4] * h1 + dd[7] * h2, d2 = dd[2] * h0 + dd[5] * h1 + dd[8] * h2;
+                if (SYM) {
+                    __hip_atomic_store(hD + 3 * i, d0, __ATOMIC_RELAXED, __HIP_MEMORY_SCOPE_AGENT);
+                    __hip_atomic_store(hD + 3 * i + 1, d1, __ATOMIC_RELAXED, __HIP_MEMORY_SCOPE_AGENT);
+                    __hip_atomic_store(hD + 3 * i + 2, d2, __ATOMIC_RELAXED, __HIP_MEMORY_SCOPE_AGENT);
+                }
+                else
+                    hD[3 * i] = d0, hD[3 * i + 1] = d1, hD[3 * i + 2] = d2;
+            }
+            else if (hD)
+                hD[3 * i] += h0, hD[3 * i + 1] += h1, hD[3 * i + 2] += h2;
+        }
+        GS_CLK_OUT();
+        return;
+    }
+    if (w != 0) return;
+    if (cnt > 0) gs_phase_b<T, DFWD, SB, true, SYM>(tri, sv, nodes, cnt, lane, diagVal, diagBlockInv, x, hD, sD);
+    GS_CLK_OUT();
diff --git a/hot_amd/csrc/mg_gs.hip b/hot_amd/csrc/mg_gs.hip
--- a/hot_amd/csrc/mg_gs.hip
+++ b/hot_amd/csrc/mg_gs.hip
@@ -136,7 +136,7 @@
     L.gs_w_ready = true;
 }
 
-template <class T, bool FWD, int SB, bool WT = false>
+template <class T, bool FWD, int SB, bool WT = false, bool WTD = false>
 __device__ __forceinline__ void gs_phase_b(const T* tri, const T* sv, const int32_t* nodes, int cnt, int lane, const T* __restrict__ diagVal, const T* __restrict__ diagBlockInv, T* x, T* hD,
     const T* ldsD = nullptr);
 
@@ -241,7 +241,7 @@
     }
 }
 
-template <class T, bool FWD, int SB, bool WT>
+template <class T, bool FWD, int SB, bool WT, bool WTD>
 __device__ __forceinline__ void gs_phase_b(const T* tri, const T* sv, const int32_t* nodes, int cnt, int lane, const T* __restrict__ diagVal, const T* __restrict__ diagBlockInv, T* x, T* hD,
     const T* ldsD)
 {
@@ -286,7 +286,12 @@
         }
         else
             x[3 * (int64_t)i] = h0, x[3 * (int64_t)i + 1] = h1, x[3 * (int64_t)i + 2] = h2;
-        if (FWD) {
+        if (FWD && WTD) {
+            __hip_atomic_store(hD + 3 * (int64_t)i, dd[0] * h0 + dd[3] * h1 + dd[6] * h2, __ATOMIC_RELAXED, __HIP_MEMORY_SCOPE_AGENT);
+            __hip_atomic_store(hD + 3 * (int64_t)i + 1, dd[1] * h0 + dd[4] * h1 + dd[7] * h2, __ATOMIC_RELAXED, __HIP_MEMORY_SCOPE_AGENT);
+            __hip_atomic_store(hD + 3 * (int64_t)i + 2, dd[2] * h0 + dd[5] * h1 + dd[8] * h2, __ATOMIC_RELAXED, __HIP_MEMORY_SCOPE_AGENT);
+        }
+        else if (FWD) {
             hD[3 * (int64_t)i] = dd[0] * h0 + dd[3] * h1 + dd[6] * h2;
             hD[3 * (int64_t)i + 1] = dd[1] * h0 + dd[4] * h1 + dd[7] * h2;
             hD[3 * (int64_t)i + 2] = dd[2] * h0 + dd[5] * h1 + dd[8] * h2;
@@ -698,6 +703,7 @@
     int sub[33];
     int color[33];
 };
+constexpr int GS_PASS_BWD = 8;
 
 #ifdef HOT_GS_CLOCKS
 __device__ unsigned long long gs_clk[34 * 8];
@@ -709,281 +715,43 @@
 #else
 #define GS_CLK(i)
 #endif
+template <class T, bool FWD, bool WINV>
+struct GsSym {
+    static constexpr bool value = FWD && WINV && sizeof(T) == 8;
+};
 template <class T, bool FWD, int SB, bool WINV = false>
 __global__ __launch_bounds__(SB * 16) void k_gs_sweep(const int32_t* __restrict__ col, const T* __restrict__ val, const uint32_t* __restrict__ ckey, const int32_t* __restrict__ gs_order,
     const int32_t* __restrict__ block_start, const T* __restrict__ diagVal, const T* __restrict__ diagBlockInv, const T* __restrict__ rhs, T* x, T* hD, GsPasses P,
     const int32_t* __restrict__ rowcnt, int* err ,
     T* unset_next ,
-    const T* __restrict__ gs_w )
-{
-    extern __shared__ __attribute__((aligned(16))) char gs_smem[];
-    constexpr int TRI = GsLds<T, SB>::TRI;
-    static_assert(!WINV || SB == 64, "the inverse images are whole-block images");
-#ifdef HOT_GS_CLOCKS
-    unsigned long long gclk_[5] = { 0, 0, 0, 0, 0 }, gt0_ = clock64();
-#endif
-    constexpr int RQ = 4, NW = SB / RQ;
-    auto ld3 = [&](int64_t j, T& x0, T& x1, T& x2) {
-        x0 = __hip_atomic_load(x + 3 * j, __ATOMIC_RELAXED, __HIP_MEMORY_SCOPE_AGENT), x1 = __hip_atomic_load(x + 3 * j + 1, __ATOMIC_RELAXED, __HIP_MEMORY_SCOPE_AGENT),
-        x2 = __hip_atomic_load(x + 3 * j + 2, __ATOMIC_RELAXED, __HIP_MEMORY_SCOPE_AGENT);
-        int spins = 0;
-        while (GsUnset<T>::is(x0) || GsUnset<T>::is(x1) || GsUnset<T>::is(x2)) {
-            __builtin_amdgcn_s_sleep(2);
-            if (++spins > (1 << 21) || ((spins & 1023) == 0 && *(volatile int*)err)) {
-                *(volatile int*)err = 1;
-                break;
-            }
-            x0 = __hip_atomic_load(x + 3 * j, __ATOMIC_RELAXED, __HIP_MEMORY_SCOPE_AGENT), x1 = __hip_atomic_load(x + 3 * j + 1, __ATOMIC_RELAXED, __HIP_MEMORY_SCOPE_AGENT),
-            x2 = __hip_atomic_load(x + 3 * j + 2, __ATOMIC_RELAXED, __HIP_MEMORY_SCOPE_AGENT);
-        }
-    };
-    T* tri = (T*)gs_smem;
-    T* sv = tri + (WINV ? GsWinv<T>::img_elems : 9 * TRI);
-    int32_t* nodes = (int32_t*)(sv + 3 * SB);
-    const int tid = threadIdx.x, lane = tid & 63, w = tid >> 6;
+    const T* __restrict__ gs_w , T* xb , T* ub )
+{
     int p = 0;
     while (p + 1 < P.npass && (int)blockIdx.x >= P.wg_begin[p + 1]) ++p;
-    const int b = P.block0[p] + ((int)blockIdx.x - P.wg_begin[p]);
-    const int lo = P.sub[p] * SB;
-    const int start = block_start[b] + lo, cnt = max(0, min(SB, block_start[b + 1] - start));
-    int32_t* rng = nodes + SB;
-    T* sDinv = (T*)(nodes + 5 * SB);
-    T* sD = sDinv + 9 * SB;
-    T* srhs = sD + 9 * SB;
-    if (!WINV)
-        for (int e = tid; e < 9 * TRI; e += 64 * NW) tri[e] = (T)0;
-    if (tid < SB) nodes[tid] = tid < cnt ? gs_order[start + tid] : -1;
-    __syncthreads();
-    GS_CLK(0);
-    if (WINV) {
-        constexpr int IMG_BYTES = GsWinv<T>::img_elems * (int)sizeof(T);
-        const char* wg = (const char*)(gs_w + ((size_t)b * 2 + (FWD ? 0 : 1)) * GsWinv<T>::img_elems);
-        for (int c = w; c * 1024 < IMG_BYTES; c += NW) {
-            const int off = c * 1024 + lane * 16;
-            if (off < IMG_BYTES)
-                __builtin_amdgcn_global_load_lds((const __attribute__((address_space(1))) void*)(wg + off), (__attribute__((address_space(3))) void*)((char*)tri + c * 1024), 16, 0, 0);
-        }
-    }
-    for (int e = tid; e < 9 * cnt; e += 64 * NW) {
-        const int64_t i = nodes[e / 9];
-        sDinv[e] = diagBlockInv[9 * i + e % 9];
-        if (FWD) sD[e] = diagVal[9 * i + e % 9];
-    }
-    for (int e = tid; e < 3 * cnt; e += 64 * NW) srhs[e] = rhs[3 * (int64_t)nodes[e / 3] + e % 3];
-    if (unset_next)
-        for (int e = tid; e < 3 * cnt; e += 64 * NW) gs_store_unset(unset_next + 3 * (int64_t)nodes[e / 3] + e % 3);
-    T bv[RQ][9];
-    int jj[RQ], node[RQ], kb2[RQ], ke[RQ];
-    const bool first_sub = p == 0 || P.color[p - 1] != P.color[p];
-    const bool head = FWD ? first_sub : !first_sub;
-    bool late[RQ];
-    const uint32_t prevkey = p > 0 ? ((uint32_t)P.color[p - 1] << 8) | (uint32_t)P.sub[p - 1] : 0xffffffffu;
-    if constexpr (WINV) {
-        int4 rc[RQ];
-#pragma unroll
-        for (int q = 0; q < RQ; ++q) {
-            const int ii = w + NW * q;
-            jj[q] = -1, kb2[q] = 0, ke[q] = 0, late[q] = false;
-            node[q] = ii < cnt ? __builtin_amdgcn_readfirstlane(nodes[ii]) : -1;
-#pragma unroll
-            for (int e = 0; e < 9; ++e) bv[q][e] = (T)0;
-        }
-#pragma unroll
-        for (int q = 0; q < RQ; ++q) rc[q] = node[q] >= 0 ? *(const int4*)(rowcnt + 4 * (int64_t)node[q]) : make_int4(0, 0, 0, 0);
-#pragma unroll
-        for (int q = 0; q < RQ; ++q) {
-            if (node[q] < 0) continue;
-            const int64_t i = node[q];
-            const int kbeg = FWD ? 0 : rc[q].x + rc[q].y + 1 + rc[q].z, kend = FWD ? rc[q].x : kbeg + rc[q].w;
-            kb2[q] = head ? kbeg + 64 : kbeg, ke[q] = head ? kend : kend - 64;
-            const int k = head ? kbeg + lane : kend - 64 + lane;
-            if (k >= kbeg && k < kend) {
-                jj[q] = col[i * 125 + k];
-                const T* bb = val + (i * 125 + k) * 9;
-#pragma unroll
-                for (int e = 0; e < 9; ++e) bv[q][e] = bb[e];
+    if constexpr (GsSym<T, FWD, WINV>::value) {
+        constexpr bool SYM = true;
+        if (P.color[p] & GS_PASS_BWD) {
+            const T* const rhs_b = hD;
+            T* const x_b = xb;
+            T* const hD_b = ub;
+            {
+                constexpr bool DFWD = false;
+                const T* __restrict__ rhs = rhs_b;
+                T* x = x_b;
+                T* hD = hD_b;
+                T* unset_next = nullptr;
+#include "gs_sweep_body.h"
             }
         }
-#pragma unroll
-        for (int q = 0; q < RQ; ++q)
-            if (jj[q] >= 0) {
-                const uint32_t keyj = ckey[jj[q]];
-                late[q] = (((keyj >> 28) << 8) | (((keyj & 127u) - 1u) / (uint32_t)SB)) == prevkey;
-            }
-    }
-    else
-#pragma unroll
-    for (int q = 0; q < RQ; ++q) {
-        const int ii = w + NW * q;
-        jj[q] = -1, node[q] = -1, kb2[q] = 0, ke[q] = 0, late[q] = false;
-#pragma unroll
-        for (int e = 0; e < 9; ++e) bv[q][e] = (T)0;
-        if (ii < cnt) {
-            const int i = nodes[ii];
-            node[q] = i;
-            const int po = rowcnt[4 * i], pi = rowcnt[4 * i + 1], fi = rowcnt[4 * i + 2], fo = rowcnt[4 * i + 3];
-            const int kbeg = FWD ? 0 : po + pi + 1, kend = FWD ? po + pi : po + pi + 1 + fi + fo;
-            const int ibeg = FWD ? po : kbeg, iend = FWD ? po + pi : kbeg + fi;
-            kb2[q] = head ? kbeg + 64 : kbeg, ke[q] = head ? kend : kend - 64;
-            rng[ii] = kb2[q], rng[SB + ii] = ke[q];
-            const int k = head ? kbeg + lane : kend - 64 + lane;
-            if (k >= kbeg && k < kend) {
-                const int j = col[(int64_t)i * 125 + k];
-                const T* bb = val + ((int64_t)i * 125 + k) * 9;
-#pragma unroll
-                for (int e = 0; e < 9; ++e) bv[q][e] = bb[e];
-                jj[q] = j;
-                const uint32_t keyj = ckey[j];
-                late[q] = (((keyj >> 28) << 8) | (((keyj & 127u) - 1u) / (uint32_t)SB)) == prevkey;
-                if (k >= ibeg && k < iend) {
-                    const int l = (int)(keyj & 127u) - 1 - lo;
-                    if (l >= 0 && l < SB) {
-                        if (!WINV) {
-                            const int idx = FWD ? gs_tri_fwd<SB>(ii, l) : gs_tri_bwd(ii, l);
-                            gs_store_tri<T>(tri, TRI, idx, diagBlockInv + 9 * (int64_t)i, bv[q]);
-                        }
-                        jj[q] = -1;
-                    }
-                }
-            }
-        }
-    }
-    __syncthreads();
-    GS_CLK(1);
-    auto is_late = [&](uint32_t keyj) { return (((keyj >> 28) << 8) | (((keyj & 127u) - 1u) / (uint32_t)SB)) == prevkey; };
-    bool tail_late[RQ];
-#pragma unroll
-    for (int q = 0; q < RQ; ++q) {
-        const int ii = w + NW * q;
-        tail_late[q] = false;
-        if (ii >= cnt) continue;
-        const int i = WINV ? node[q] : nodes[ii], kt0 = WINV ? kb2[q] : rng[ii], kt1 = WINV ? ke[q] : rng[SB + ii];
-        T e0 = 0, e1 = 0, e2 = 0;
-        if (jj[q] >= 0 && !late[q]) {
-            const int64_t j = jj[q];
-            T x0, x1, x2;
-            ld3(j, x0, x1, x2);
-            e0 = bv[q][0] * x0 + bv[q][3] * x1 + bv[q][6] * x2;
-            e1 = bv[q][1] * x0 + bv[q][4] * x1 + bv[q][7] * x2;
-            e2 = bv[q][2] * x0 + bv[q][5] * x1 + bv[q][8] * x2;
-        }
-        bool tl = false;
-        for (int k = kt0 + lane; k < kt1; k += 64) {
-            const int j = col[(int64_t)i * 125 + k];
-            const T* bb = val + ((int64_t)i * 125 + k) * 9;
-            const uint32_t keyj = ckey[j], keyi = ckey[i];
-            const int l = (int)(keyj & 127u) - 1 - lo;
-            if ((keyj >> 7) == (keyi >> 7) && l >= 0 && l < SB) {
-                if (!WINV) {
-                    const int idx = FWD ? gs_tri_fwd<SB>(ii, l) : gs_tri_bwd(ii, l);
-                    T bt[9];
-#pragma unroll
-                    for (int e = 0; e < 9; ++e) bt[e] = bb[e];
-                    gs_store_tri<T>(tri, TRI, idx, diagBlockInv + 9 * (int64_t)i, bt);
-                }
-            }
-            else if (is_late(keyj))
-                tl = true;
-            else {
-                T x0, x1, x2;
-                ld3(j, x0, x1, x2);
-                e0 += bb[0] * x0 + bb[3] * x1 + bb[6] * x2;
-                e1 += bb[1] * x0 + bb[4] * x1 + bb[7] * x2;
-                e2 += bb[2] * x0 + bb[5] * x1 + bb[8] * x2;
-            }
-        }
-        tail_late[q] = __ballot(tl) != 0ull;
-        e0 = wave_sum(e0), e1 = wave_sum(e1), e2 = wave_sum(e2);
-        if (lane == 0) srhs[3 * ii] -= e0, srhs[3 * ii + 1] -= e1, srhs[3 * ii + 2] -= e2;
-    }
-    GS_CLK(2);
-    const T* val_again = val;
-    asm volatile("" : "+s"(val_again));
-#pragma unroll
-    for (int q = 0; q < RQ; ++q) {
-        const int ii = w + NW * q;
-        if (ii >= cnt) continue;
-        const int i = WINV ? node[q] : nodes[ii], kt0 = WINV ? kb2[q] : rng[ii], kt1 = WINV ? ke[q] : rng[SB + ii];
-        T s0 = 0, s1 = 0, s2 = 0;
-        if (jj[q] >= 0 && late[q]) {
-            const int64_t j = jj[q];
-            const T* bb = val_again + ((int64_t)i * 125 + (head ? kt0 - 64 : kt1) + lane) * 9;
-            T bl[9];
-#pragma unroll
-            for (int e = 0; e < 9; ++e) bl[e] = bb[e];
-            T x0, x1, x2;
-            ld3(j, x0, x1, x2);
-            s0 = bl[0] * x0 + bl[3] * x1 + bl[6] * x2;
-            s1 = bl[1] * x0 + bl[4] * x1 + bl[7] * x2;
-            s2 = bl[2] * x0 + bl[5] * x1 + bl[8] * x2;
-        }
-        if (tail_late[q]) {
-            for (int k = kt0 + lane; k < kt1; k += 64) {
-                const int j = col[(int64_t)i * 125 + k];
-                const T* bb = val + ((int64_t)i * 125 + k) * 9;
-                const uint32_t keyj = ckey[j], keyi = ckey[i];
-                const int l = (int)(keyj & 127u) - 1 - lo;
-                if (!((keyj >> 7) == (keyi >> 7) && l >= 0 && l < SB) && is_late(keyj)) {
-                    T x0, x1, x2;
-                    ld3(j, x0, x1, x2);
-                    s0 += bb[0] * x0 + bb[3] * x1 + bb[6] * x2;
-                    s1 += bb[1] * x0 + bb[4] * x1 + bb[7] * x2;
-                    s2 += bb[2] * x0 + bb[5] * x1 + bb[8] * x2;
-                }
-            }
-        }
-        s0 = wave_sum(s0), s1 = wave_sum(s1), s2 = wave_sum(s2);
-        if (lane == 0) gs_store_rhs<T>(sv, ii, sDinv + 9 * ii, srhs[3 * ii] - s0, srhs[3 * ii + 1] - s1, srhs[3 * ii + 2] - s2);
-    }
-    __syncthreads();
-    GS_CLK(3);
-#ifdef HOT_GS_CLOCKS
-#define GS_CLK_OUT() \
-    do { \
-        GS_CLK(4); \
-        if (tid == 0) \
-            for (int i = 0; i < 5; ++i) atomicAdd(&gs_clk[p * 8 + i], gclk_[i]); \
-        if (tid == 0) atomicAdd(&gs_clk[p * 8 + 7], 1ull); \
-    } while (0)
-#else
-#define GS_CLK_OUT()
-#endif
-    if (WINV) {
-        const bool cin = lane < cnt;
-        const T ac0 = cin ? sv[3 * lane] : (T)0, ac1 = cin ? sv[3 * lane + 1] : (T)0, ac2 = cin ? sv[3 * lane + 2] : (T)0;
-        T h0 = 0, h1 = 0, h2 = 0;
-#pragma unroll
-        for (int k = 0; k < 4; ++k) {
-            const int rr = 4 * w + k;
-            if (rr >= cnt) break;
-            const bool act = FWD ? lane < rr : (lane > rr && cin);
-            const int idx = act ? gs_winv_idx<FWD>(rr, lane) : TRI - 1;
-            T Lw[9];
-#pragma unroll
-            for (int e = 0; e < 9; ++e) Lw[e] = tri[e * TRI + idx];
-            T t0 = Lw[0] * ac0 + Lw[3] * ac1 + Lw[6] * ac2, t1 = Lw[1] * ac0 + Lw[4] * ac1 + Lw[7] * ac2, t2 = Lw[2] * ac0 + Lw[5] * ac1 + Lw[8] * ac2;
-            t0 = wave_sum(t0), t1 = wave_sum(t1), t2 = wave_sum(t2);
-            if (lane == k) h0 = sv[3 * rr] + t0, h1 = sv[3 * rr + 1] + t1, h2 = sv[3 * rr + 2] + t2;
-        }
-        const int me = 4 * w + lane;
-        if (lane < 4 && me < cnt) {
-            const int64_t i = nodes[me];
-            __hip_atomic_store(x + 3 * i, h0, __ATOMIC_RELAXED, __HIP_MEMORY_SCOPE_AGENT);
-            __hip_atomic_store(x + 3 * i + 1, h1, __ATOMIC_RELAXED, __HIP_MEMORY_SCOPE_AGENT);
-            __hip_atomic_store(x + 3 * i + 2, h2, __ATOMIC_RELAXED, __HIP_MEMORY_SCOPE_AGENT);
-            if (FWD) {
-                const T* dd = sD + 9 * me;
-                hD[3 * i] = dd[0] * h0 + dd[3] * h1 + dd[6] * h2, hD[3 * i + 1] = dd[1] * h0 + dd[4] * h1 + dd[7] * h2, hD[3 * i + 2] = dd[2] * h0 + dd[5] * h1 + dd[8] * h2;
-            }
-            else if (hD)
-                hD[3 * i] += h0, hD[3 * i + 1] += h1, hD[3 * i + 2] += h2;
-        }
-        GS_CLK_OUT();
-        return;
-    }
-    if (w != 0) return;
-    if (cnt > 0) gs_phase_b<T, FWD, SB, true>(tri, sv, nodes, cnt, lane, diagVal, diagBlockInv, x, hD, sD);
-    GS_CLK_OUT();
+        else {
+            constexpr bool DFWD = true;
+#include "gs_sweep_body.h"
+        }
+    }
+    else {
+        constexpr bool SYM = false, DFWD = FWD;
+#include "gs_sweep_body.h"
+    }
 }
 
 template <class T>
@@ -1320,19 +1088,37 @@
     };
 
     if (tmp_marked && !plan.marks) zero(n3, hdu), tmp_marked = false;
-    GsPasses PF{}, PB{};
+    GsPasses PF{}, PB{}, PS{};
+    bool sym_chain = false;
     if (plan.path == GsPlan::CHAINED) {
-        auto add = [&](GsPasses& P, int c, int h) {
+        auto add = [&](GsPasses& P, int c, int h, int dir) {
             int b0 = L.color_block_begin[c], nb = L.color_block_begin[c + 1] - b0;
             if (nb <= 0) return;
-            P.block0[P.npass] = b0, P.sub[P.npass] = h, P.color[P.npass] = c, P.wg_begin[P.npass + 1] = P.wg_begin[P.npass] + nb;
+            P.block0[P.npass] = b0, P.sub[P.npass] = h, P.color[P.npass] = c | dir, P.wg_begin[P.npass + 1] = P.wg_begin[P.npass] + nb;
             ++P.npass;
         };
         for (int c = 0; c < 8; ++c)
-            for (int h = 0; h < nsub; ++h) add(PF, c, h);
+            for (int h = 0; h < nsub; ++h) add(PF, c, h, 0);
         for (int c = 7; c >= 0; --c)
-            for (int h = nsub - 1; h >= 0; --h) add(PB, c, h);
-    }
+            for (int h = nsub - 1; h >= 0; --h) add(PB, c, h, 0);
+        sym_chain = GsSym<T, true, true>::value && plan.winv && !ab_flag("HOT_GS_NO_SYM_CHAIN") && max_colour_blocks(L) <= 256 && PF.npass > 0 && PF.npass + PB.npass <= 33;
+        if (sym_chain) {
+            for (int c = 0; c < 8; ++c) add(PS, c, 0, 0);
+            for (int c = 7; c >= 0; --c) add(PS, c, 0, GS_PASS_BWD);
+        }
+    }
+    auto chained_sym_sweep = [&]() {
+        const bool all_marked = tmp_marked && du == L.du.p && dAu == L.dAu.p;
+        if (!tmp_marked) HOT_LAUNCH(this, "gs_fill_unset", k_gs_fill_unset<T>, div_up(n3, 256), 256, 0, n3, hdu);
+        tmp_marked = false;
+        if (!all_marked) {
+            HOT_LAUNCH(this, "gs_fill_unset", k_gs_fill_unset<T>, div_up(n3, 256), 256, 0, n3, du);
+            HOT_LAUNCH(this, "gs_fill_unset", k_gs_fill_unset<T>, div_up(n3, 256), 256, 0, n3, dAu);
+        }
+        const int grid = PS.wg_begin[PS.npass];
+        HOT_LAUNCH(this, lname("gs_forward", L.id).c_str(), (k_gs_sweep<T, true, 64, true>), grid, 16 * 64, (GsLds<T, 64>::bytes + 21 * 64 * sizeof(T) + 128), L.col.p, L.val.p, L.ckey.p, L.gs_order.p,
+            L.gs_block_start.p, L.diagVal.p, L.diagBlockInv.p, r, hdu, dAu, PS, L.rowcnt.p, (int*)(hscal + 250), (T*)nullptr, L.gs_w.p, du, u);
+    };
     bool du_marked = false;
     auto chained_sweep = [&](bool fwd) {
         const GsPasses& P = fwd ? PF : PB;
@@ -1349,7 +1135,7 @@
 #define HOT_GS_CASE(F, S, ...)                                                                                                                                         \
     HOT_LAUNCH(this, lname(nm, L.id).c_str(), (k_gs_sweep<T, F, S, ##__VA_ARGS__>), grid, 16 * S, (GsLds<T, S>::bytes + 21 * S * sizeof(T) + 128), L.col.p, L.val.p, L.ckey.p, L.gs_order.p, L.gs_block_start.p, \
         L.diagVal.p, L.diagBlockInv.p, rhs, xx, hD, P, rc, (int*)(hscal + 250), \
-        fwd ? du : (T*)nullptr, L.gs_w.p)
+        fwd ? du : (T*)nullptr, L.gs_w.p, (T*)nullptr, (T*)nullptr)
         du_marked = fwd;
         if (plan.winv) {
             if (fwd)
@@ -1397,11 +1183,19 @@
     for (; iterations--;) {
         prof.count(lname("gs_symsweeps", L.id));
         if (rank_local) zero(n3, hdu), zero(n3, du);
-        half_sweep(true);
+        if (sym_chain) {
+            chained_sym_sweep();
 #ifdef HOT_GS_CLOCKS
-        if (plan.path == GsPlan::CHAINED) clk_report("forward");
-#endif
-        half_sweep(false);
+            clk_report("symmetric");
+#endif
+        }
+        else {
+            half_sweep(true);
+#ifdef HOT_GS_CLOCKS
+            if (plan.path == GsPlan::CHAINED) clk_report("forward");
+#endif
+            half_sweep(false);
+        }
 #ifdef HOT_GSC_CLOCKS
         if (plan.path == GsPlan::COLOUR && L.id == 0) {
             static int sweeps = 0;
diff --git a/hot_amd/csrc/mg_solve.hip b/hot_amd/csrc/mg_solve.hip
--- a/hot_amd/csrc/mg_solve.hip
+++ b/hot_amd/csrc/mg_solve.hip
@@ -216,12 +216,17 @@
 }
 template <class T>
 __global__ __launch_bounds__(256) void k_apmv_sub(const int32_t* __restrict__ apc, const T* __restrict__ apv, const T* __restrict__ e, T* __restrict__ r, int n, const uint8_t* __restrict__ own,
-    T* unset )
+    T* unset ,
+    T* unset2 = nullptr, T* unset3 = nullptr )
 {
     const int lane = threadIdx.x & 63;
     const int row = xcd_block() * 4 + (threadIdx.x >> 6);
     if (row >= n) return;
-    if (unset && lane < 3) gs_store_unset(unset + 3 * (int64_t)row + lane);
+    if (unset && lane < 3) {
+        gs_store_unset(unset + 3 * (int64_t)row + lane);
+        if (unset2) gs_store_unset(unset2 + 3 * (int64_t)row + lane);
+        if (unset3) gs_store_unset(unset3 + 3 * (int64_t)row + lane);
+    }
     if (own && !own[row]) return;
     const int j = nt_load(apc + (int64_t)row * 64 + lane);
     const int slot = __popcll(__ballot(j >= 0) & ((1ull << lane) - 1ull));
@@ -647,11 +652,16 @@
 
 template <class T>
 __global__ void k_restrict(const int32_t* __restrict__ child, const T* __restrict__ fine, T* coarse, int nc, const uint8_t* __restrict__ coarse_own, const uint8_t* __restrict__ fine_own,
-    T* unset , T* zero_out = nullptr )
+    T* unset , T* zero_out = nullptr ,
+    T* unset2 = nullptr, T* unset3 = nullptr )
 {
     int e = blockIdx.x * blockDim.x + threadIdx.x;
     if (e >= 3 * nc) return;
-    if (unset) gs_store_unset(unset + e);
+    if (unset) {
+        gs_store_unset(unset + e);
+        if (unset2) gs_store_unset(unset2 + e);
+        if (unset3) gs_store_unset(unset3 + e);
+    }
     if (zero_out) zero_out[e] = (T)0;
     int I = e / 3, d = e - 3 * I;
     if (coarse_own && !coarse_own[I]) return;
@@ -711,7 +721,8 @@
         return;
     }
     T* mark = gs_marks_wanted(level + 1) ? C.tmp.p : (T*)nullptr;
-    HOT_LAUNCH(this, "restrict", k_restrict<T>, div_up(3 * (size_t)C.n, 256), 256, 0, C.child.p, fine, coarse, C.n, (const uint8_t*)nullptr, (const uint8_t*)nullptr, mark, zero_coarse);
+    HOT_LAUNCH(this, "restrict", k_restrict<T>, div_up(3 * (size_t)C.n, 256), 256, 0, C.child.p, fine, coarse, C.n, (const uint8_t*)nullptr, (const uint8_t*)nullptr, mark, zero_coarse,
+        mark ? C.du.p : (T*)nullptr, mark ? C.dAu.p : (T*)nullptr);
     unset_level = mark ? level + 1 : -1;
 }
 template <class T>
@@ -1022,7 +1033,8 @@
         else
         {
             T* mark = gs_marks_wanted(level) ? L.tmp.p : (T*)nullptr;
-            HOT_LAUNCH(this, lname("apmv", L.id).c_str(), k_apmv_sub<T>, xcd_grid(div_up(L.n, 4)), 256, 0, L.apc.p, L.apv.p, levels[level + 1]->sol.p, L.residual.p, L.n, L.mask(), mark);
+            HOT_LAUNCH(this, lname("apmv", L.id).c_str(), k_apmv_sub<T>, xcd_grid(div_up(L.n, 4)), 256, 0, L.apc.p, L.apv.p, levels[level + 1]->sol.p, L.residual.p, L.n, L.mask(), mark,
+                mark ? L.du.p : (T*)nullptr, mark ? L.dAu.p : (T*)nullptr);
             unset_level = mark ? level : -1;
         }
         if (L.part && !halo_mode() && smoother_kind(level) != 5)
```

Result: no change. 3.022 ms/iter, median of 2 (-0.2%).
